# foollh/PicoPose

Hardware: AMD Instinct MI355X
Metric: image-crops/sec (224x224, 162 templates) (higher is better)
Workload: dtype f32 tensors; networks: f32 operands split into 2 f16 terms (22 bits) on f16 MFMA with f32 accumulate; stage-1 contraction: f16 MFMA operands, f32 accumulate, exact f32 re-evaluation of near-ties; PnP f64

## Files before the change

include/picopose_hip.h:

```cpp
#ifndef PICOPOSE_HIP_H
#define PICOPOSE_HIP_H

#include <stddef.h>
#include <stdint.h>

#ifdef __cplusplus
extern "C" {
#endif

#define PP_OK 0
#define PP_EINVAL (-1)
#define PP_EWORKSPACE (-2)
#define PP_ELAUNCH (-3)

#define PP_MATCH_EXACT 0
#define PP_MATCH_FAST 1

const char* pp_strerror(int code);
int pp_version(void);

int pp_prof_enable(int max_records);
int pp_prof_collect(float* out_ms, int max_out, int* count);
int pp_prof_gemm_enable(int max_records);
int pp_prof_gemm_collect(double* ms, double* flops, int* launches);
// ... 97 lines not shown
    const void* B_hl;
    float b_scale;
    const void* A_hl;
    long long a_hl_bytes, b_hl_bytes;
    void* C_hl;
    int ldc_h;
    int c_relu;
    const float* alpha_dev;
    const float* alpha_dev2;
    int ksplit;
    int ks_rows;
    int grp_rows;
    long long grp_b_bytes;
} PpGemmDesc;

int pp_gemm(const PpGemmDesc* desc, void* stream);
int pp_split_f16x3(const float* w, long long n, void* hl, float* scale, void* stream);
int pp_split_weights_ws(const float* w, long long n, int terms, void* out, float* scale2, float* partials, void* stream);
int pp_split_activation(const float* x, long long batch_stride, int B, int P, int row_stride, int C, int relu,
                        void* hl, void* stream);
int pp_split_activation_ld(const float* x, long long batch_stride, int B, int P, int row_stride, int C, int relu,
                           void* hl, int ld_h, void* stream);
int pp_pow2_scale_ws(const float* x, long long n, float* scale2, float* partials, void* stream);
int pp_split_scaled_t(const float* x, long long rows, int ld, int C, const float* scale, void* out, int terms, void* stream);
int pp_split_transpose_t(const float* x, long long rows, int cols, int ld, const float* scale, void* out, int terms, void* stream);
int pp_split_transpose_ld(const float* x, long long rows, int cols, int ld, const float* scale, void* out, long long ld_out, int terms,
                          void* stream);
int pp_im2col_t_operand(const float* x, int B, int H, int W, int C, int ksize, int stride, int pad, void* out, int terms, void* stream);
int pp_sum_slices(const float* part, int S, int M, int N, const float* bias, int act, float* out, void* stream);
int pp_hl_patch_columns(const float* x, int ld_x, int c, long long rows, void* hl, int ld_h, int col0, void* stream);

int pp_split_weights_t(const float* w, long long n, int terms, void* out, float* scale, void* stream);
int pp_split_activation_t(const float* x, long long batch_stride, int B, int P, int row_stride, int C, int relu, void* out,
                          int ld_h, int terms, void* stream);
int pp_hl_patch_columns_t(const float* x, int ld_x, int c, long long rows, void* out, int ld_h, int col0, int terms, void* stream);
int pp_layernorm_t(const float* x, const float* gamma, const float* beta, int rows, int C, float eps, float* y, void* out, int terms,
                   void* stream);
int pp_resize_bilinear_nhwc_t(const float* in, int B, int H, int W, int C, int Ho, int Wo, float mul, void* out, int terms,
                              void* stream);
int pp_resize_bilinear_nhwc_dual(const float* in, int B, int H, int W, int C, int Ho, int Wo, float mul, float* out, void* out_operand,
                                 int terms, void* stream);
int pp_warp_nhwc_t(const float* feat, int feat_batch, const float* flow, int B, int H, int W, int C, int ld_flow, void* out,
                   int ld_h, int terms, void* stream);
int pp_attention_t(const void* qkv_operand, int terms, int B, int T, int heads, int head_dim, float scale, float* out,
                   void* out_operand, void* stream);

int pp_attention(const float* qkv, int B, int T, int heads, int head_dim, float scale, float* out, void* stream);
int pp_attention_split(const float* qkv, int B, int T, int heads, int head_dim, float scale, float* out, void* out_hl,
                       void* stream);
int pp_attention_ex(const float* qkv, int B, int T, int heads, int head_dim, float scale, int prec, float* out, void* out_hl,
                    void* stream);
int pp_attention_hl(const void* qkv_hl, int B, int T, int heads, int head_dim, float scale, float* out, void* out_hl,
                    void* stream);
int pp_attention_train(const float* qkv, int B, int T, int heads, int head_dim, float scale, float* out, float* lse2, void* stream);
int pp_attention_backward(const float* qkv, const float* out, const float* dout, const float* lse2, const float* gpair, int B, int T,
                          int heads, int head_dim, float scale, float* Dws, float* dqkv, void* stream);

int pp_layernorm(const float* x, const float* gamma, const float* beta, int rows, int C, float eps,
                 float* y, void* stream);
int pp_layernorm_split(const float* x, const float* gamma, const float* beta, int rows, int C, float eps, float* y,
                       void* hl, void* stream);
int pp_softmax_rows(float* x, int rows, int n, int ld, void* stream);
int pp_groupnorm_nhwc(const float* x, const float* gamma, const float* beta, int B, int HW, int C,
                      int groups, float eps, int relu, float* y, void* stream);
int pp_transpose_batched(const float* in, long long in_batch_stride, int B, int R, int C, float* out,
                         long long out_batch_stride, int ld_out, int col_off, void* stream);
int pp_assemble_tokens(const float* patches, const float* cls_token, const float* pos, int B, int T, int C,
                       float* tokens, void* stream);
int pp_normalize_rows(const float* x, int rows, int n, float eps, float* y, void* stream);

int pp_resize_bilinear_nhwc(const float* in, int B, int H, int W, int C, int Ho, int Wo, float mul,
                            float* out, void* stream);
int pp_resize_bilinear_nhwc_hl(const float* in, int B, int H, int W, int C, int Ho, int Wo, float mul, void* out_hl,
                               void* stream);
int pp_warp_nhwc(const float* feat, int feat_batch, const float* flow, int B, int H, int W, int C, int ld_flow,
                 float* out, int ld_out, void* stream);
int pp_warp_nhwc_hl(const float* feat, int feat_batch, const float* flow, int B, int H, int W, int C, int ld_flow,
                    void* out_hl, int ld_h, void* stream);
int pp_avgpool2_nhwc(const float* in, int B, int H, int W, int C, float* out, void* stream);
int pp_gather_rows(const float* src, const long long* index, long long n_src_rows, long long row_floats, int n, float* dst,
                   void* stream);
int pp_bank_rows_to_tokens(const float* bank, long long n_bank_rows, int C, int P, const long long* index, int n, float* tokens, int ld,
                           int T, int skip, void* stream);

int pp_crop_resize_normalize(const unsigned char* image, int H, int W, const unsigned char* mask, int y1, int y2, int x1,
                             int x2, int S, int rgb_mask_flag, const double* mean3, const double* std3, float* out_rgb,
                             float* out_mask, void* stream);
int pp_depth_points_nearest(const float* depth_m, int H, int W, int y1, int y2, int x1, int x2, int P, float fx, float fy,
                            float cx, float cy, float* out_pts, void* stream);
int pp_corr_lookup_nhwc(const float* f1, int ld_f1, const float* f2_l0, const float* f2_l1, const float* f2_l2,
                        int f2_batch, const float* flow, int B, int H, int W, int C, int levels, int radius,
                        int ld_flow, float* out, int ld_out, void* stream);
int pp_corr_lookup_nhwc_ex(const float* f1, int ld_f1, const float* f2_l0, const float* f2_l1, const float* f2_l2,
                           int f2_batch, const float* flow, int B, int H, int W, int C, int levels, int radius,
                           int ld_flow, int prec, float* out, int ld_out, void* stream);

int pp_conv_narrow_hl(const void* x_hl, int ld_x, int B, int H, int W, int C, const float* weight, const float* bias, int ksize,
                      int n_out, const float* residual, float* out, void* stream);
int pp_conv_narrow_f32(const float* x, int ld_x, int B, int H, int W, int C, const float* weight, const float* bias, int ksize,
                       int n_out, const float* residual, float* out, void* stream);

int pp_winograd_input_f32(const float* x, int ld_x, long long batch_stride, int B, int H, int W, int C, int relu, float* U, void* stream);
int pp_winograd_weight_f32(const float* w, int Cout, int Cin, int ldw, float* V, void* stream);
int pp_winograd_output_f32(const float* Y, int B, int H, int W, int Cout, const float* bias, int act, const float* residual,
                           const float* residual2, float* out, int ldc, void* stream);

int pp_winograd4_input_hl(const void* x_hl, int ld_x, long long batch_stride, int B, int H, int W, int C, int relu, void* U_hl, long long P_pad,
                          void* stream);
int pp_winograd4_weight_f32(const float* w, int Cout, int Cin, int ldw, float* V, void* stream);
int pp_winograd4_output(const float* Y, int ld_y, int B, int H, int W, int Cout, const float* bias, int act, const float* residual,
                        const float* residual2, float* out, int ldc, void* out_hl, int ld_h, int c_relu, long long P_pad, void* stream);

int pp_winograd4_chain(const float* Y, int ld_y, int B, int H, int W, int C, const float* bias, int act, int c_relu, void* U_hl, long long P_pad,
                       void* stream);

int pp_winograd_chain_f32(const float* Y, int B, int H, int W, int C, const float* bias, int act, int relu_next, float* U, void* stream);

int pp_set_saturation_word(unsigned int* word);

int pp_saturation_take(unsigned int* word, unsigned int* slot, void* stream);


int pp_corr_lookup_nhwc_hl(const void* f1_hl, int ld_f1, const void* f2_hl_l0, const void* f2_hl_l1, const void* f2_hl_l2,
                           int f2_batch, const float* flow, int B, int H, int W, int C, int levels, int radius, int ld_flow,
                           float* out, int ld_out, void* stream);

int pp_pnp_ransac(const float* tar_pts_2d, const float* src_pts_3d, const float* K, const float* tem_pose,
                  const int64_t* tar_pts, const int64_t* src_pts, int P, int H, int W, int N, int iterations,
                  float reproj_threshold, double* rot, double* tvec, double* inlier_ratio, int32_t* success,
                  int32_t* num_points, void* stream);

int pp_pnp_ransac_debug(const float* tar_pts_2d, const float* src_pts_3d, const float* K, const float* tem_pose,
                        const int64_t* tar_pts, const int64_t* src_pts, int P, int H, int W, int N, int iterations,
                        float reproj_threshold, double* rot, double* tvec, double* inlier_ratio, int32_t* success,
                        int32_t* num_points, double* refit_branches, void* stream);

int pp_pnp_ransac_refine(const float* tar_pts_2d, const float* src_pts_3d, const float* K, const float* tem_pose,
                         const int64_t* tar_pts, const int64_t* src_pts, int P, int H, int W, int N, int iterations,
                         float reproj_threshold, int max_iters, double eps, double* rot, double* tvec, double* inlier_ratio,
                         int32_t* success, int32_t* num_points, double* rms_before, double* rms_after, int32_t* lm_iterations,
                         uint8_t* inlier_mask, void* stream);

int pp_pnp_refine_lm(const double* object_points, const double* image_points, const int32_t* count, const double* K,
                     const double* rot_init, const double* tvec_init, int P, int Nmax, int max_iters, double eps, double* rot,
                     double* tvec, double* rms_before, double* rms_after, int32_t* lm_iterations, void* stream);

int pp_rgbd_ransac(const float* tar_pts_2d, const float* src_pts_3d, const float* K, const float* tem_pose,
                   const int64_t* tar_pts, const int64_t* src_pts, int P, int H, int W, int N,
                   const float* depth, int n_images, int dH, int dW, const int32_t* image_index,
                   const float* inlier_dist, int iterations,
                   double* rot, double* tvec, double* inlier_ratio, int32_t* success,
                   int32_t* num_points, int32_t* num_listed, double* rms, uint8_t* inlier_mask, void* stream);

size_t pp_train_keypoints_workspace_bytes(int B);
int pp_train_keypoints(const float* src_mask, const float* tar_mask, int mask_h, int mask_w, const float* src_depth,
                       const float* tar_depth, int depth_h, int depth_w, const float* src_Minv, const float* tar_Minv,
                       const float* src_M, const float* tar_M, const float* src_Kinv, const float* tar_Kinv, const float* src_K,
                       const float* tar_K, const float* T_src2tar, const float* T_tar2src, int B, float* src_pts, float* tar_pts,
                       void* workspace, size_t workspace_bytes, void* stream);
size_t pp_batchnorm_train_workspace_bytes(int rows, int C);
int pp_batchnorm_train(const float* x, const float* gamma, const float* beta, int rows, int C, float eps, float momentum,
                       float* running_mean, float* running_var, int relu, const float* residual, const float* residual2, float* y,
                       void* workspace, size_t workspace_bytes, void* stream);
int pp_gather_normalize_rows(const float* src, long long row_stride, const int64_t* index, int n, int C, float eps, float* out,
                             void* stream);
int pp_xent_diag_rows(const float* logits, int n, int ld, float scale, float* row_loss, void* stream);
// ... 210 lines not shown
```

picopose_amd/_lib.py:

```python
import ctypes
import os
import re

from .build import LIB

_HEADER = os.path.join(os.path.dirname(os.path.abspath(__file__)), "..", "include", "picopose_hip.h")

PP_OK = 0
PP_MATCH_EXACT = 0
PP_MATCH_FAST = 1
PP_BANK_F32 = 0
PP_BANK_F16 = 1

_lib = None


class PpGemmDesc(ctypes.Structure):
    _fields_ = [
        ("A", ctypes.c_void_p), ("B", ctypes.c_void_p), ("C", ctypes.c_void_p), ("bias", ctypes.c_void_p),
        ("gamma", ctypes.c_void_p), ("residual", ctypes.c_void_p), ("residual2", ctypes.c_void_p),
        ("M", ctypes.c_int), ("N", ctypes.c_int), ("K", ctypes.c_int),
        ("lda", ctypes.c_int), ("ldb", ctypes.c_int), ("ldc", ctypes.c_int), ("b_kn", ctypes.c_int),
        ("batch0", ctypes.c_int), ("batch1", ctypes.c_int),
        ("a_bs0", ctypes.c_longlong), ("a_bs1", ctypes.c_longlong), ("b_bs0", ctypes.c_longlong),
# ... 44 lines not shown
            )
        import torch

        L = ctypes.CDLL(LIB)
        c = ctypes
        vp, i32, f32, sz = c.c_void_p, c.c_int, c.c_float, c.c_size_t
        L.pp_strerror.restype = c.c_char_p
        L.pp_strerror.argtypes = [i32]
        L.pp_version.restype = i32
        L.pp_prof_enable.argtypes = [i32]
        L.pp_prof_collect.argtypes = [c.POINTER(f32), i32, c.POINTER(i32)]
        L.pp_prof_gemm_enable.argtypes = [i32]
        L.pp_prof_gemm_collect.argtypes = [c.POINTER(c.c_double), c.POINTER(c.c_double), c.POINTER(i32)]
        L.pp_prof_gemm_records.argtypes = [i32, c.POINTER(i32), c.POINTER(f32), c.POINTER(c.c_double), c.POINTER(i32)]
        L.pp_prof_gemm_records2.argtypes = [i32, c.POINTER(i32), c.POINTER(f32), c.POINTER(c.c_double), c.POINTER(c.c_double), c.POINTER(i32)]
        L.pp_gemm_tune_save.argtypes = [c.c_char_p]
        L.pp_gemm_tune_load.argtypes = [c.c_char_p]
        L.pp_gemm_tune_entries.argtypes = []
        L.pp_gemm_generic_epilogue.argtypes = [i32]
        L.pp_stage1_workspace_bytes.argtypes = [i32, i32, i32, c.POINTER(sz)]
        L.pp_stage1_scores.argtypes = [vp, vp, vp, i32, i32, i32, i32, i32, i32, f32, vp, sz, vp, vp, vp]
        L.pp_stage1_scores_ex.argtypes = [vp, i32, vp, vp, i32, i32, i32, i32, i32, i32, f32, vp, sz, vp, vp, vp]
        L.pp_topk.argtypes = [vp, i32, i32, i32, vp, vp, vp]
        L.pp_stage1_match.argtypes = [vp, vp, vp, i32, i32, i32, i32, i32, i32, i32, f32, vp, sz,
                                      vp, vp, vp, vp, vp]
        L.pp_stage1_match_ex.argtypes = [vp, i32, vp, vp, i32, i32, i32, i32, i32, i32, i32, f32, vp, sz, vp, vp, vp, vp, vp]
        L.pp_stage1_indexed_workspace_bytes.argtypes = [i32, i32, i32, c.POINTER(sz)]
        L.pp_stage1_scores_indexed.argtypes = [vp, i32, vp, i32, vp, vp, i32, i32, i32, i32, i32, i32, f32, vp, sz, vp, vp, vp]
        L.pp_stage1_match_indexed.argtypes = [vp, i32, vp, i32, vp, vp, i32, i32, i32, i32, i32, i32, i32, f32, vp, sz, vp, vp, vp,
                                              vp, vp]
        L.pp_similarity_volume.argtypes = [vp, vp, vp, i32, i32, i32, i32, vp, vp]
        L.pp_calc_pred_Ms.argtypes = [vp, vp, vp, vp, vp, vp, i32, f32, vp, vp]
        L.pp_pose_recovery_2d.argtypes = [vp, vp, vp, vp, vp, vp, i32, vp, vp]
        L.pp_init_correspondences.argtypes = [vp, vp, i32, i32, i32, vp, vp, vp]
        L.pp_stage3_correspondences.argtypes = [vp, vp, i32, i32, i32, f32, vp, vp, vp]
        L.pp_gather_valid.argtypes = [vp, vp, i32, i32, i32, i32, i32, vp, vp, vp]
        L.pp_gemm.argtypes = [c.POINTER(PpGemmDesc), vp]
        L.pp_split_f16x3.argtypes = [vp, c.c_longlong, vp, vp, vp]
        L.pp_split_activation.argtypes = [vp, c.c_longlong, i32, i32, i32, i32, i32, vp, vp]
        L.pp_split_activation_ld.argtypes = [vp, c.c_longlong, i32, i32, i32, i32, i32, vp, i32, vp]
        L.pp_conv_narrow_hl.argtypes = [vp, i32, i32, i32, i32, i32, vp, vp, i32, i32, vp, vp, vp]
        L.pp_conv_narrow_f32.argtypes = [vp, i32, i32, i32, i32, i32, vp, vp, i32, i32, vp, vp, vp]
        L.pp_winograd_input_f32.argtypes = [vp, i32, c.c_longlong, i32, i32, i32, i32, i32, vp, vp]
        L.pp_winograd_weight_f32.argtypes = [vp, i32, i32, i32, vp, vp]
        L.pp_winograd_output_f32.argtypes = [vp, i32, i32, i32, i32, vp, i32, vp, vp, vp, i32, vp]
        L.pp_winograd4_input_hl.argtypes = [vp, i32, c.c_longlong, i32, i32, i32, i32, i32, vp, c.c_longlong, vp]
        L.pp_winograd4_weight_f32.argtypes = [vp, i32, i32, i32, vp, vp]
        L.pp_winograd4_output.argtypes = [vp, i32, i32, i32, i32, i32, vp, i32, vp, vp, vp, i32, vp, i32, i32, c.c_longlong, vp]
        L.pp_winograd4_chain.argtypes = [vp, i32, i32, i32, i32, i32, vp, i32, i32, vp, c.c_longlong, vp]
        L.pp_winograd_chain_f32.argtypes = [vp, i32, i32, i32, i32, vp, i32, i32, vp, vp]
        L.pp_set_saturation_word.argtypes = [vp]
        L.pp_saturation_take.argtypes = [vp, vp, vp]
        L.pp_split_weights_t.argtypes = [vp, c.c_longlong, i32, vp, vp, vp]
        L.pp_split_weights_ws.argtypes = [vp, c.c_longlong, i32, vp, vp, vp, vp]
        L.pp_split_activation_t.argtypes = [vp, c.c_longlong, i32, i32, i32, i32, i32, vp, i32, i32, vp]
        L.pp_hl_patch_columns_t.argtypes = [vp, i32, i32, c.c_longlong, vp, i32, i32, i32, vp]
        L.pp_layernorm_t.argtypes = [vp, vp, vp, i32, i32, f32, vp, vp, i32, vp]
        L.pp_resize_bilinear_nhwc_t.argtypes = [vp, i32, i32, i32, i32, i32, i32, f32, vp, i32, vp]
        L.pp_resize_bilinear_nhwc_dual.argtypes = [vp, i32, i32, i32, i32, i32, i32, f32, vp, vp, i32, vp]
        L.pp_warp_nhwc_t.argtypes = [vp, i32, vp, i32, i32, i32, i32, i32, vp, i32, i32, vp]
        L.pp_attention_t.argtypes = [vp, i32, i32, i32, i32, i32, f32, vp, vp, vp]
        L.pp_sum_slices.argtypes = [vp, i32, i32, i32, vp, i32, vp, vp]
        L.pp_hl_patch_columns.argtypes = [vp, i32, i32, c.c_longlong, vp, i32, i32, vp]
        L.pp_warp_nhwc_hl.argtypes = [vp, i32, vp, i32, i32, i32, i32, i32, vp, i32, vp]
        L.pp_attention.argtypes = [vp, i32, i32, i32, i32, f32, vp, vp]
        L.pp_attention_split.argtypes = [vp, i32, i32, i32, i32, f32, vp, vp, vp]
        L.pp_attention_ex.argtypes = [vp, i32, i32, i32, i32, f32, i32, vp, vp, vp]
        L.pp_attention_hl.argtypes = [vp, i32, i32, i32, i32, f32, vp, vp, vp]
        L.pp_attention_train.argtypes = [vp, i32, i32, i32, i32, f32, vp, vp, vp]
        L.pp_attention_backward.argtypes = [vp, vp, vp, vp, vp, i32, i32, i32, i32, f32, vp, vp, vp]
        L.pp_layernorm.argtypes = [vp, vp, vp, i32, i32, f32, vp, vp]
        L.pp_layernorm_split.argtypes = [vp, vp, vp, i32, i32, f32, vp, vp, vp]
        L.pp_softmax_rows.argtypes = [vp, i32, i32, i32, vp]
        L.pp_groupnorm_nhwc.argtypes = [vp, vp, vp, i32, i32, i32, i32, f32, i32, vp, vp]
        L.pp_transpose_batched.argtypes = [vp, c.c_longlong, i32, i32, i32, vp, c.c_longlong, i32, i32, vp]
        L.pp_assemble_tokens.argtypes = [vp, vp, vp, i32, i32, i32, vp, vp]
        L.pp_normalize_rows.argtypes = [vp, i32, i32, f32, vp, vp]
        L.pp_resize_bilinear_nhwc.argtypes = [vp, i32, i32, i32, i32, i32, i32, f32, vp, vp]
        L.pp_resize_bilinear_nhwc_hl.argtypes = [vp, i32, i32, i32, i32, i32, i32, f32, vp, vp]
        L.pp_warp_nhwc.argtypes = [vp, i32, vp, i32, i32, i32, i32, i32, vp, i32, vp]
        L.pp_avgpool2_nhwc.argtypes = [vp, i32, i32, i32, i32, vp, vp]
        L.pp_gather_rows.argtypes = [vp, vp, c.c_longlong, c.c_longlong, i32, vp, vp]
        L.pp_bank_rows_to_tokens.argtypes = [vp, c.c_longlong, i32, i32, vp, i32, vp, i32, i32, i32, vp]
        L.pp_depth_points_nearest.argtypes = [vp, i32, i32, i32, i32, i32, i32, i32, f32, f32, f32, f32, vp, vp]
        L.pp_crop_resize_normalize.argtypes = [vp, i32, i32, vp, i32, i32, i32, i32, i32, i32, c.POINTER(c.c_double),
                                               c.POINTER(c.c_double), vp, vp, vp]
        L.pp_corr_lookup_nhwc.argtypes = [vp, i32, vp, vp, vp, i32, vp, i32, i32, i32, i32, i32, i32, i32, vp, i32, vp]
        L.pp_corr_lookup_nhwc_ex.argtypes = [vp, i32, vp, vp, vp, i32, vp, i32, i32, i32, i32, i32, i32, i32, i32, vp, i32, vp]
        L.pp_corr_lookup_nhwc_hl.argtypes = [vp, i32, vp, vp, vp, i32, vp, i32, i32, i32, i32, i32, i32, i32, vp, i32, vp]
        L.pp_pnp_ransac.argtypes = [vp, vp, vp, vp, vp, vp, i32, i32, i32, i32, i32, f32, vp, vp, vp, vp, vp, vp]
        L.pp_pnp_ransac_debug.argtypes = [vp, vp, vp, vp, vp, vp, i32, i32, i32, i32, i32, f32, vp, vp, vp, vp, vp, vp, vp]
        L.pp_pnp_ransac_refine.argtypes = [vp, vp, vp, vp, vp, vp, i32, i32, i32, i32, i32, f32, i32, c.c_double] + [vp] * 10
        L.pp_pnp_refine_lm.argtypes = [vp] * 6 + [i32, i32, i32, c.c_double] + [vp] * 6
        L.pp_rgbd_ransac.argtypes = [vp] * 6 + [i32] * 4 + [vp, i32, i32, i32, vp, vp, i32] + [vp] * 9
        L.pp_train_keypoints_workspace_bytes.restype = sz
        L.pp_train_keypoints_workspace_bytes.argtypes = [i32]
        L.pp_train_keypoints.argtypes = [vp, vp, i32, i32, vp, vp, i32, i32] + [vp] * 10 + [i32, vp, vp, vp, sz, vp]
        L.pp_batchnorm_train_workspace_bytes.restype = sz
        L.pp_batchnorm_train_workspace_bytes.argtypes = [i32, i32]
        L.pp_batchnorm_train.argtypes = [vp, vp, vp, i32, i32, f32, f32, vp, vp, i32, vp, vp, vp, vp, sz, vp]
        L.pp_gather_normalize_rows.argtypes = [vp, c.c_longlong, vp, i32, i32, f32, vp, vp]
        L.pp_xent_diag_rows.argtypes = [vp, i32, i32, f32, vp, vp]
        L.pp_flow_loss_blocks.argtypes = []
        L.pp_flow_loss_sums.argtypes = [vp, vp, vp, i32, i32, i32, f32, vp, vp]
        ll = c.c_longlong
        L.pp_colsum_workspace_bytes.restype = sz
        L.pp_colsum_workspace_bytes.argtypes = [ll, i32]
        L.pp_colsum.argtypes = [vp, ll, i32, i32, vp, vp, sz, vp]
        L.pp_act_forward.argtypes = [vp, ll, i32, vp, vp]
        L.pp_act_backward.argtypes = [vp, vp, ll, i32, vp, vp]
        L.pp_elementwise.argtypes = [i32, vp, vp, ll, i32, vp, vp]
        L.pp_layernorm_backward.argtypes = [vp, vp, vp, i32, i32, f32, vp, vp, vp]
        L.pp_groupnorm_backward_nhwc.argtypes = [vp, vp, vp, vp, i32, i32, i32, i32, f32, i32, vp, vp, vp, vp]
        L.pp_softmax_backward_rows.argtypes = [vp, vp, ll, i32, vp, vp]
        L.pp_xent_diag_backward.argtypes = [vp, i32, i32, f32, vp, vp, vp]
        L.pp_normalize_rows_backward.argtypes = [vp, ll, vp, vp, i32, i32, f32, vp, vp]
        L.pp_scatter_add_rows.argtypes = [vp, vp, i32, i32, vp, vp]
        L.pp_im2col_nhwc.argtypes = [vp, i32, i32, i32, i32, i32, i32, i32, vp, vp]
        L.pp_col2im_nhwc.argtypes = [vp, i32, i32, i32, i32, i32, i32, i32, vp, vp]
        L.pp_simvol_backward.argtypes = [vp, vp, vp, i32, i32, i32, vp, vp]
        L.pp_im2col_t_nhwc.argtypes = [vp, i32, i32, i32, i32, i32, i32, i32, vp, vp]
        L.pp_pow2_scale.argtypes = [vp, ll, vp, vp]
        L.pp_pow2_scale_ws.argtypes = [vp, ll, vp, vp, vp]
        L.pp_split_scaled_t.argtypes = [vp, ll, i32, i32, vp, vp, i32, vp]
        L.pp_split_transpose_t.argtypes = [vp, ll, i32, i32, vp, vp, i32, vp]
        L.pp_split_transpose_ld.argtypes = [vp, ll, i32, i32, vp, vp, ll, i32, vp]
        L.pp_im2col_t_operand.argtypes = [vp, i32, i32, i32, i32, i32, i32, i32, vp, i32, vp]
        L.pp_split_with_scale_t.argtypes = [vp, ll, i32, vp, vp, vp]
        L.pp_batchnorm_train_backward_workspace_bytes.restype = sz
        L.pp_batchnorm_train_backward_workspace_bytes.argtypes = [ll, i32]
        L.pp_batchnorm_train_backward.argtypes = [vp, vp, vp, vp, ll, i32, f32, i32, vp, vp, vp, vp, sz, vp]
        L.pp_resize_bilinear_backward_nhwc.argtypes = [vp, i32, i32, i32, i32, i32, i32, f32, vp, vp]
        L.pp_avgpool2_backward_nhwc.argtypes = [vp, i32, i32, i32, i32, i32, vp, vp]
        L.pp_warp_backward_nhwc.argtypes = [vp, vp, vp, i32, i32, i32, i32, i32, vp, vp, vp]
        L.pp_corr_lookup_backward_nhwc.argtypes = [vp, vp, vp, vp, i32, i32, i32, i32, i32, i32, i32, i32, vp, vp, vp, vp]
        L.pp_warp_backward_nhwc_fixed.argtypes = [vp, vp, vp, i32, i32, i32, i32, i32, vp, vp, vp]
        L.pp_corr_lookup_backward_nhwc_fixed.argtypes = [vp, vp, vp, vp, i32, i32, i32, i32, i32, i32, i32, i32, vp, vp, vp, vp]
        L.pp_fixed_to_float.argtypes = [vp, ll, vp, vp]
        L.pp_flow_loss_backward.argtypes = [vp, vp, vp, i32, i32, i32, f32, vp, vp, vp, vp, vp]
        L.pp_adam_workspace_bytes.argtypes = [c.POINTER(PpAdamTensor), i32, c.POINTER(sz)]
        L.pp_adam_multi_tensor.argtypes = [c.POINTER(PpAdamTensor), i32, vp, i32, i32, vp, sz, vp]
        L.pp_augment_execute.argtypes = [vp, vp, ll, vp, ll, vp, i32, vp, i32, vp, c.POINTER(i32), i32, vp, vp, ll, vp, vp]
        L.pp_augment_resize.argtypes = [vp, vp, ll, vp, i32, i32, i32, c.POINTER(c.c_double), c.POINTER(c.c_double), vp, vp, vp]
        L.pp_depth_u16_scaled.argtypes = [vp, ll, i32, vp, vp, vp]
        L.pp_depth_u16_template.argtypes = [vp, ll, vp, vp]
        L.pp_detections_crop.argtypes = [vp, i32, i32, vp, i32, vp, vp, c.POINTER(i32), c.POINTER(i32), i32, i32, i32,
                                         c.POINTER(c.c_double), c.POINTER(c.c_double), vp, vp, vp]
        L.pp_render_workspace_bytes.argtypes = [i32, i32, i32, i32, c.POINTER(sz)]
        L.pp_render_views.argtypes = [vp, i32, vp, vp, i32, vp, vp, i32, f32, f32, f32, f32, i32, i32, f32, vp, sz, vp, vp, vp, vp, vp, vp]
        L.pp_texture_mips_bytes.argtypes = [i32, i32, c.POINTER(sz), c.POINTER(i32)]
        L.pp_texture_build_mips.argtypes = [vp, i32, i32, vp, sz, vp]
        L.pp_render_views_textured.argtypes = [vp, i32, vp, vp, i32, vp, vp, i32, i32, vp, i32, f32, f32, f32, f32, i32, i32, f32, vp, sz,
                                               vp, vp, vp, vp, vp, vp]
        L.pp_vertex_normals.argtypes = [vp, i32, vp, i32, vp, vp, vp, vp]
        L.pp_render_views_lit.argtypes = [vp, i32, vp, vp, i32, vp, vp, vp, i32, i32, vp, i32, f32, f32, f32, f32, i32, i32, f32, vp, sz,
                                          vp, vp, vp, vp, vp, vp, i32, f32, i32, vp, vp, vp, i32, vp]
        L.pp_template_extents.argtypes = [vp, i32, i32, i32, vp, vp, vp]
        L.pp_templates_crop.argtypes = [vp, vp, i32, i32, i32, i32, vp, vp, f32, f32, f32, f32, i32, i32, i32,
                                        c.POINTER(c.c_double), c.POINTER(c.c_double), vp, vp, vp, vp]
        L.pp_pose_errors_workspace_bytes.argtypes = [i32, i32, i32, i32, c.POINTER(sz)]
        L.pp_pose_errors.argtypes = [vp] * 10 + [i32] + [vp] * 7 + [i32, i32, vp, sz] + [vp] * 7
        L.pp_vsd_workspace_bytes.argtypes = [ll, ll, c.POINTER(sz)]
        scene = c.POINTER(PpScene)
        L.pp_vsd_errors.argtypes = [scene, vp, vp, vp, vp, i32, vp, f32, vp, i32, vp, sz, vp, vp, vp, vp, vp]
        L.pp_depth_refine_workspace_bytes.argtypes = [ll, ll, ll, c.POINTER(sz)]
        L.pp_depth_refine.argtypes = [scene, vp, vp, vp, vp, vp, i32, f32, i32, f32, f32, f32, f32, f32, vp, sz,
# ... 37 lines not shown
```

picopose_amd/csrc/pp_gemm.hip:

```cpp

#include <hip/hip_runtime.h>
#include <stdint.h>
#include <stdio.h>
#include <stdlib.h>
#include <atomic>
#include <mutex>
#include <string>
#include <unordered_map>
#include "../../include/picopose_hip.h"
#include "pp_common.h"
#include "pp_gemm_dev.h"
#include "pp_gemm_u.h"

static std::mutex g_tune_mu;
static std::unordered_map<std::string, int> g_tune_best;
static int g_tune_loaded = 0;

static int tune_load_locked(const char* path) {
    FILE* f = fopen(path, "r");
    if (!f) return -1;
    char key[192];
    int cfg, n = 0;
    while (fscanf(f, "%191s %d", key, &cfg) == 2) {
        g_tune_best[key] = cfg;
// ... 1068 lines not shown
        PpGemmDesc g = d;
        g.grp_rows = d.M;
        g.grp_b_bytes = d.b_bs0 * 4;
        g.M = d.M * d.batch0;
        g.batch0 = 1;
        if (pp_gemm_f_ok(g)) d = g;
    }
    if (d.A_hl && d.B_hl && d.batch0 > 1 && d.batch1 == 1 && d.conv_kh == 0 && !d.b_kn && d.shuffle_r == 0 && !d.residual && !d.residual2 &&
        d.ksplit <= 1 && !d.C_hl && d.M % 256 == 0 && d.a_bs0 == (long long)d.M * d.lda && d.c_bs0 == (long long)d.M * d.ldc &&
        (long long)d.M * d.batch0 < (1LL << 31) && d.b_bs0 >= 0 && d.b_bs0 % 8 == 0) {
        d.grp_rows = d.M;
        d.grp_b_bytes = d.b_bs0 * (d.prec == PP_PREC_F16 ? 2 : 4);
        d.M *= d.batch0;
        d.batch0 = 1;
    }
    const long long z = v.z = (long long)d.batch0 * d.batch1;
    const bool f16 = d.prec == PP_PREC_F16;
    const int terms = v.terms = f16 ? 1 : 2;
    const bool split = v.split = d.prec == PP_PREC_F16X3 && vec;
    const bool asplit = v.asplit = d.A_hl != nullptr;
    if (f16 && !asplit) return PP_EINVAL;
    if (asplit) {
        const bool ok = d.B_hl && (d.prec == PP_PREC_F16X3 || f16) && z == 1 && !d.b_kn && !d.relu_in &&
                        d.K % 8 == 0 && d.lda % 8 == 0 && d.ldb % 8 == 0 && d.b_scale > 0.f &&
                        (d.conv_kh == 0 || (d.conv_cin % 8 == 0 && d.conv_bstride % 8 == 0)) &&
                        ((uintptr_t)d.A_hl % 16 == 0) && ((uintptr_t)d.B_hl % 16 == 0);
        if (!ok) return PP_EINVAL;
        pp_gemm_extents(d, 2 * terms, d.a_hl_bytes, d.b_hl_bytes);
        if (d.a_hl_bytes >= 0xFFFFFF00LL || d.b_hl_bytes >= 0xFFFFFF00LL) return PP_EINVAL;
    }
    d.ks_rows = 0;
    if (d.ksplit > 1) {
        if (!asplit || d.conv_kh != 0 || d.M % 256 != 0 || d.K % (64 * d.ksplit) != 0 || d.bias || d.gamma || d.residual || d.residual2 ||
            d.act != 0 || d.C_hl || d.shuffle_r != 0 || !d.C || (long long)d.M * d.ksplit >= (1LL << 31))
            return PP_EINVAL;
        d.ks_rows = d.M;
        d.M *= d.ksplit;
        d.K /= d.ksplit;
    }
    if (d.B_hl && (d.b_kn || d.ldb % 8 != 0 || d.K % 8 != 0 || z != 1 || !(d.b_scale > 0.f))) return PP_EINVAL;
    if (d.B_hl && !split && !f16) {
        if (d.alpha_dev || d.alpha_dev2) return PP_EINVAL;
        d.B_hl = nullptr;
    }
    v.fvec = f_engine_on && !asplit && !split && vec && z == 1 && pp_gemm_f_ok(d);
    if (v.fvec) pp_gemm_extents(d, 4, d.a_hl_bytes, d.b_hl_bytes);
    v.u_vec = asplit && pp_gemm_u_vec_ok(d);
    v.h_shape = v.u_vec && pp_gemm_uh_shape_ok(d, terms);
    return PP_OK;
}

static int tail_rows(const GemmView& v, int big_bn, int cus) {
    const PpGemmDesc& d = v.d;
    if (!((v.asplit || v.fvec) && d.conv_kh == 0 && d.shuffle_r == 0 && d.ks_rows == 0 && d.grp_rows == 0 && v.z == 1)) return 0;
    const long long gx = (d.N + big_bn - 1) / big_bn, gy = (d.M + 255) / 256, tiles = gx * gy, full = tiles / cus;
    if (full < 1 || tiles % cus == 0) return 0;
    const long long r = full * cus / gx * 256;
    return (r > 0 && r < d.M && d.M - r >= 128) ? (int)r : 0;
}

enum { GE_U, GE_UH, GE_F, GE_FLY, GE_R1 };
struct GemmPlan {
    int engine;
    int cfg;
    int tile;
    int amode;
    bool vec;
    int tail_rows;
};

static GemmPlan gemm_plan(const GemmView& v, int cfg, int cus) {
    const PpGemmDesc& d = v.d;
    GemmPlan p{};
    if (cfg == 9 || cfg == 10) {
        p.tail_rows = cfg == 10 || d.N > 128 ? tail_rows(v, cfg == 9 ? 256 : 128, cus) : 0;
        cfg = cfg == 9 ? 5 : 4;
    }
    if (v.asplit) {
        cfg = cfg == 3 ? 4 : (cfg == 1 || cfg == 7 || cfg == 8) ? 0 : cfg;
        if (cfg == 6 && !(v.h_shape && d.N > 128)) cfg = 5;
        if (cfg == 5 && d.N <= 128) cfg = 4;
        if (!v.u_vec && cfg != 2) cfg = 0;
        p.engine = cfg == 6 ? GE_UH : GE_U;
        p.tile = cfg == 5 ? PP_U_256x256 : cfg == 4 ? PP_U_256x128 : cfg == 2 ? PP_U_128x64 : PP_U_128x128;
        p.amode = cfg == 6 ? 1 : pp_gemm_u_mode(d, v.terms);
        p.vec = v.u_vec;
    } else if (v.fvec && (cfg >= 3 || d.grp_rows != 0)) {
        if (cfg < 3) cfg = 3;
        const int mode = pp_gemm_f_mode(d);
        if (mode == 2 && (cfg == 5 || cfg == 7)) cfg = 4;
        p.engine = GE_F;
        p.tile = cfg == 7 ? PP_F_256x192 : cfg == 5 ? PP_U_256x256 : cfg == 4 ? PP_U_256x128 : cfg == 3 ? PP_U_128x128 : PP_U_128x64;
        p.amode = 16 + mode;
    } else {
        p.engine = v.split ? GE_FLY : GE_R1;
        p.amode = 8 + (v.vec ? 1 : 0) + (v.split ? 2 : 0);
        p.vec = v.vec;
    }
    p.cfg = cfg;
    return p;
}

static int gemm_r1_launch(const GemmPlan& p, const PpGemmDesc& d, long long z, hipStream_t st) {
    const bool narrow = p.cfg == 2, occ2 = p.cfg == 0;
    void (*k)(PpGemmDesc);
    if (p.engine == GE_FLY && d.B_hl) k = narrow ? gemm_f16x3_kernel<1, 4, true> : occ2 ? gemm_f16x3_kernel<2, 2, true> : gemm_f16x3_kernel<2, 3, true>;
    else if (p.engine == GE_FLY) k = narrow ? gemm_f16x3_kernel<1, 4, false> : occ2 ? gemm_f16x3_kernel<2, 2, false> : gemm_f16x3_kernel<2, 3, false>;
    else if (!p.vec) k = narrow ? gemm_kernel<false, 1, 2> : gemm_kernel<false, 2, 2>;
    else k = narrow ? gemm_kernel<true, 1, 4> : occ2 ? gemm_kernel<true, 2, 2> : gemm_kernel<true, 2, 3>;
    const dim3 grid((d.N + (narrow ? 63 : 127)) / (narrow ? 64 : 128), (unsigned)((d.M + BM - 1) / BM), (unsigned)z);
    void* args[] = {(void*)&d};
    (void)hipLaunchKernel((const void*)k, grid, dim3(256), args, 0, st);
    return PP_OK;
}

static int gemm_launch(const GemmPlan& p, const GemmView& v, int cus, hipStream_t st) {
    auto one = [&](const PpGemmDesc& d, int tile) {
        switch (p.engine) {
            case GE_U: return (v.terms == 2 ? pp_gemm_u_launch_t2 : pp_gemm_u_launch_t1)(d, tile, p.amode, p.vec, cus, st);
            case GE_UH: return pp_gemm_uh_launch(d, v.terms, cus, st);
            case GE_F: return pp_gemm_f_launch(d, tile, p.amode - 16, cus, st);
            default: return gemm_r1_launch(p, d, v.z, st);
        }
    };
    if (p.tail_rows == 0) return one(v.d, p.tile);
    auto rows = [&](int r0, int m) {
        PpGemmDesc t = v.d;
        t.M = m;
        const size_t eb = v.terms == 1 ? 2 : 4;
        if (t.A_hl) t.A_hl = (const char*)t.A_hl + (size_t)r0 * t.lda * eb;
        if (t.A) t.A += (size_t)r0 * t.lda;
        if (t.C) t.C += (size_t)r0 * t.ldc;
        if (t.C_hl) t.C_hl = (char*)t.C_hl + (size_t)r0 * t.ldc_h * eb;
        if (t.residual) t.residual += (size_t)r0 * t.ldc;
        if (t.residual2) t.residual2 += (size_t)r0 * t.ldc;
        pp_gemm_extents(t, (int)eb, t.a_hl_bytes, t.b_hl_bytes);
        return t;
    };
    const int rc = one(rows(0, p.tail_rows), p.tile);
    return rc != PP_OK ? rc : one(rows(p.tail_rows, v.d.M - p.tail_rows), PP_U_128x128);
}

static int tune_candidates(const GemmView& v, int cus, int* c) {
    static const int tail_env = [] { const char* e = getenv("PP_GEMM_TAIL_SPLIT"); return e ? (e[0] == '1' ? 1 : 0) : -1; }();
    const PpGemmDesc& d = v.d;
    const bool tail_on = tail_env == 1, tail_on_f = tail_env != 0;
    const long long t4 = (long long)((d.M + 255) / 256) * ((d.N + 127) / 128), t5 = (long long)((d.M + 255) / 256) * ((d.N + 255) / 256);
    int n = 0;
    if (v.asplit) {
        c[n++] = 0;
        c[n++] = 2;
        if (t4 >= cus / 2) c[n++] = 4;
        if (t5 >= cus / 2 && d.N > 128) c[n++] = 5;
        if (t5 >= cus / 2 && d.N > 128 && v.h_shape) c[n++] = 6;
        if (tail_on && d.N > 128 && tail_rows(v, 256, cus)) c[n++] = 9;
        if (tail_on && tail_rows(v, 128, cus)) c[n++] = 10;
    } else if (v.fvec) {
        c[n++] = 6;
        if (d.N > 64) c[n++] = 3;
        if (t4 >= cus / 2 && d.N > 64) c[n++] = 4;
        if (t5 >= cus / 2 && d.N > 128) c[n++] = 5;
        if ((d.N + 191) / 192 * 192 - d.N < (d.N + 127) / 128 * 128 - d.N && (long long)((d.M + 255) / 256) * ((d.N + 191) / 192) >= cus / 2) c[n++] = 7;
        if (tail_on_f && d.N > 128 && tail_rows(v, 256, cus)) c[n++] = 9;
        if (tail_on_f && d.N > 64 && tail_rows(v, 128, cus)) c[n++] = 10;
    } else {
        for (int i = 0; i < (v.vec ? 3 : 2); ++i) c[n++] = v.vec ? i : (i == 0 ? 0 : 2);
    }
    return n;
}

static int gemm_tune(const GemmView& v, const char* key, int cus, hipStream_t st) {
    static const bool dbg = getenv("PP_GEMM_DEBUG") != nullptr;
    hipEvent_t e0, e1;
    PP_CHECK_HIP(hipEventCreate(&e0));
    PP_CHECK_HIP(hipEventCreate(&e1));
    int cands[12];
    const int nc = tune_candidates(v, cus, cands);
    GemmPlan plans[12];
    float ms[12];
    for (int i = 0; i < nc; ++i) {
        plans[i] = gemm_plan(v, cands[i], cus);
        ms[i] = 1e30f;
        (void)gemm_launch(plans[i], v, cus, st);
    }
    for (int rep = 0; rep < 4; ++rep)
        for (int i = 0; i < nc; ++i) {
            (void)hipEventRecord(e0, st);
            for (int k = 0; k < 4; ++k) (void)gemm_launch(plans[i], v, cus, st);
            (void)hipEventRecord(e1, st);
            (void)hipEventSynchronize(e1);
            float t = 0.f;
            (void)hipEventElapsedTime(&t, e0, e1);
            ms[i] = t < ms[i] ? t : ms[i];
        }
    (void)hipEventDestroy(e0);
    (void)hipEventDestroy(e1);
    int best = 0;
    for (int i = 0; i < nc; ++i) {
        if (dbg) fprintf(stderr, "[pp_gemm] autotune %s cfg %d: %.4f ms\n", key, cands[i], ms[i]);
        if (ms[i] < ms[best]) best = i;
    }
    g_tune_best[key] = cands[best];
    const int rc = gemm_launch(plans[best], v, cus, st);
    return rc != PP_OK ? rc : pp_last_launch();
}

extern "C" {

int pp_gemm_generic_epilogue(int on) {
    if (on != 0 && on != 1) return PP_EINVAL;
    return g_epi_generic.exchange(on);
}

int pp_gemm(const PpGemmDesc* desc, void* stream) {
    GemmView v;
    if (const int rc = gemm_normalise(desc, v); rc != PP_OK) return rc;
    const PpGemmDesc& d = v.d;
    hipStream_t st = (hipStream_t)stream;
    const int cus = pp_cu_count();
    int cfg = v.fvec ? (d.N <= 64 ? 6 : 3) : (d.N <= 64 ? 2 : 0);
    bool pinned = false;
    if (const char* f = getenv("PP_GEMM_FORCE_CFG")) {
        const int fc = atoi(f);
        if (((fc == 9 || fc == 10) && (v.asplit || v.fvec)) || (fc >= 0 && fc <= 8 && (v.asplit || fc <= 2 || (v.fvec && fc <= 7)))) {
            cfg = fc;
            pinned = true;
        }
    }
    const bool alias = d.C != nullptr && (d.residual == d.C || d.residual2 == d.C);
    static const bool tune = [] { const char* e = getenv("PP_GEMM_AUTOTUNE"); return !(e && e[0] == '0'); }();
    if (!pinned && tune && !alias && (d.N > 64 || v.fvec)) {
        [[maybe_unused]] static const bool env_loaded = [] {
            if (const char* p = getenv("PP_GEMM_TUNE_FILE")) {
                std::lock_guard<std::mutex> lock(g_tune_mu);
                (void)tune_load_locked(p);
            }
            return true;
        }();
        char key[160];
        snprintf(key, sizeof key, "%d.%d.%d.%d.%d.%lld.%d.%d.%d.%d.%d.%d", d.M, d.N, d.K, (int)v.vec, d.b_kn, v.z, d.conv_kh,
                 d.conv_cin, d.conv_stride, d.conv_h, d.shuffle_r,
                 (int)v.split + 2 * (d.B_hl != nullptr) + 4 * (int)v.asplit + 8 * (int)(v.terms == 1) + 16 * (int)v.fvec);
        std::lock_guard<std::mutex> lock(g_tune_mu);
        auto it = g_tune_best.find(key);
        if (it == g_tune_best.end()) return gemm_tune(v, key, cus, st);
        cfg = it->second;
    }
    const GemmPlan p = gemm_plan(v, cfg, cus);
    PpGemmProf* gp = pp_gemm_prof_state();
    const bool rec = gp->capacity > 0 && gp->count < gp->capacity;
    if (rec) (void)hipEventRecord(gp->ev[2 * gp->count], st);
    const int rc = gemm_launch(p, v, cus, st);
    if (rec) {
        (void)hipEventRecord(gp->ev[2 * gp->count + 1], st);
        gp->flops[gp->count] = 2.0 * d.M * d.N * d.K * (double)v.z;
        const double eb = 2.0 * v.terms, ea = v.asplit ? eb : 4.0, ew = (v.asplit || d.B_hl) ? eb : 4.0;
        const long long per = (long long)d.conv_ho * d.conv_wo;
        const double a_el = d.conv_kh != 0 ? (double)((d.M + per - 1) / per) * d.conv_h * d.conv_w * d.conv_cin
                                           : (double)d.M * d.K;
        const double mn = (double)d.M * d.N;
        gp->bytes[gp->count] = (double)v.z * (a_el * ea + (double)d.N * d.K * ew * (d.grp_rows ? d.M / d.grp_rows : 1) + (d.C ? mn * 4.0 : 0.0) +
                                              (d.C_hl ? mn * eb : 0.0) + (d.residual ? mn * 4.0 : 0.0) + (d.residual2 ? mn * 4.0 : 0.0));
        gp->kind[gp->count] = p.engine == GE_U || p.engine == GE_UH ? 0 : 1;
        int* sh = gp->shape[gp->count];
        sh[0] = d.M, sh[1] = d.N, sh[2] = d.K, sh[3] = d.conv_kh, sh[4] = p.cfg, sh[5] = p.amode;
        gp->count++;
    }
    return rc != PP_OK ? rc : pp_last_launch();
}

int pp_gemm_tune_save(const char* path) {
    if (!path) return PP_EINVAL;
    std::lock_guard<std::mutex> lock(g_tune_mu);
    FILE* f = fopen(path, "w");
    if (!f) return PP_EINVAL;
    for (const auto& kv : g_tune_best) fprintf(f, "%s %d\n", kv.first.c_str(), kv.second);
    fclose(f);
    return (int)g_tune_best.size();
}

int pp_gemm_tune_load(const char* path) {
    if (!path) return PP_EINVAL;
    std::lock_guard<std::mutex> lock(g_tune_mu);
    const int n = tune_load_locked(path);
    return n < 0 ? PP_EINVAL : n;
}

int pp_gemm_tune_entries(void) {
    std::lock_guard<std::mutex> lock(g_tune_mu);
    return (int)g_tune_best.size();
}

int pp_layernorm(const float* x, const float* gamma, const float* beta, int rows, int C, float eps, float* y,
                 void* stream) {
    if (!x || !gamma || !beta || !y || rows <= 0 || C <= 0) return PP_EINVAL;
    launch_layernorm(x, gamma, beta, rows, C, eps, y, nullptr, (hipStream_t)stream);
    return pp_last_launch();
}

int pp_layernorm_t(const float* x, const float* gamma, const float* beta, int rows, int C, float eps, float* y,
                   void* hl, int terms, void* stream) {
    if (!x || !gamma || !beta || !hl || rows <= 0 || C <= 0 || C % 8 != 0 || (terms != 1 && terms != 2)) return PP_EINVAL;
    launch_layernorm(x, gamma, beta, rows, C, eps, y, (_Float16*)hl, (hipStream_t)stream, terms);
    return pp_last_launch();
}

int pp_layernorm_split(const float* x, const float* gamma, const float* beta, int rows, int C, float eps, float* y,
// ... 46 lines not shown
```

picopose_amd/csrc/pp_gemm_u.h:

```cpp
#ifndef PP_GEMM_U_H
#define PP_GEMM_U_H
#include <hip/hip_runtime.h>
#include "../../include/picopose_hip.h"

enum { PP_U_128x64 = 0, PP_U_128x128 = 1, PP_U_256x128 = 2, PP_U_256x256 = 3, PP_F_256x192 = 4  };

int pp_gemm_u_mode(const PpGemmDesc& d, int terms);
int pp_gemm_u_launch_t1(const PpGemmDesc& d, int tile, int mode, bool vec, int cus, hipStream_t st);
int pp_gemm_u_launch_t2(const PpGemmDesc& d, int tile, int mode, bool vec, int cus, hipStream_t st);
bool pp_gemm_uh_shape_ok(const PpGemmDesc& d, int terms);
bool pp_gemm_u_vec_ok(const PpGemmDesc& d);
int pp_gemm_epi_kind(const PpGemmDesc& d);
int pp_gemm_uh_launch(const PpGemmDesc& d, int terms, int cus, hipStream_t st);
bool pp_gemm_f_ok(const PpGemmDesc& d);
int pp_gemm_f_mode(const PpGemmDesc& d);
int pp_gemm_f_launch(const PpGemmDesc& d, int tile, int mode, int cus, hipStream_t st);

static inline void pp_gemm_extents(const PpGemmDesc& d, int eb, long long& a, long long& b) {
    const long long per = (long long)d.conv_ho * d.conv_wo;
    a = eb * (d.conv_kh != 0 ? ((d.M + per - 1) / per - 1) * d.conv_bstride + (long long)d.conv_h * d.conv_w * d.lda : (long long)(d.M - 1) * d.lda + d.K);
    b = eb * ((long long)(d.N - 1) * d.ldb + d.K + (d.grp_rows != 0 ? (long long)(d.M / d.grp_rows - 1) * d.b_bs0 : 0));
}
#endif
```

picopose_amd/csrc/pp_gemm_u_kernel.h:

```cpp
#ifndef PP_GEMM_U_KERNEL_H
#define PP_GEMM_U_KERNEL_H
#include <hip/hip_runtime.h>
#include <stdint.h>
#include <type_traits>
#include "pp_gemm_dev.h"
#include "pp_gemm_u.h"

typedef __attribute__((address_space(3))) void* lds_ptr_t;
#ifdef PP_STUDY_OFFMASK
#define PP_STUDY_OFF(x) ((x) & (unsigned)(PP_STUDY_OFFMASK))
#else
#define PP_STUDY_OFF(x) (x)
#endif

#ifndef PP_U1_BAND_ROWS
#define PP_U1_BAND_ROWS 4
#endif

template <int BM_, int BN_, int WM_, int WN_, int S_, int OCC_, int PREF_ = 0, int B3_ = 0>
struct TileCfg {
    static constexpr int BM = BM_, BN = BN_, WM = WM_, WN = WN_, S = S_, OCC = OCC_;
    static constexpr bool PREF = PREF_ != 0;
    static constexpr bool B3 = B3_ != 0;
    static constexpr int NW = WM_ * WN_;
// ... 758 lines not shown
    int cab = 0;
    load_a(fa0, 0, -1, 0);
    load_b(fb0, 0, 0);
    int cur = 0;
    const float descale = pp_alpha(d) / (PP_A_SCALE * d.b_scale);
    for (int tile = first; tile < chunk1; tile += nxw) {
#pragma unroll
        for (int i = 0; i < MI; ++i)
#pragma unroll
            for (int j = 0; j < NJ; ++j) acc[i][j] = f32x4{0.f, 0.f, 0.f, 0.f};
#define PP_H_STEP(DX, NDX, NAB)                                                                                       \
        {                                                                                                             \
            load_b(fb1, cur, 1);                                                                                      \
            load_a(fa1, cab, DX, 1);                                                                                  \
            mma_unit(fa0, fb0, 0, 0);                                                                                 \
            __builtin_amdgcn_sched_barrier(0);                                                                        \
            mma_unit(fa0, fb1, 0, 1);                                                                                 \
            __builtin_amdgcn_sched_barrier(0);                                                                        \
            load_a(fa0, cab, DX, 2);                                                                                  \
            mma_unit(fa1, fb0, 1, 0);                                                                                 \
            __builtin_amdgcn_sched_barrier(0);                                                                        \
            mma_unit(fa1, fb1, 1, 1);                                                                                 \
            __builtin_amdgcn_sched_barrier(0);                                                                        \
            load_a(fa1, cab, DX, 3);                                                                                  \
            mma_unit(fa0, fb0, 2, 0);                                                                                 \
            __builtin_amdgcn_sched_barrier(0);                                                                        \
            mma_unit(fa0, fb1, 2, 1);                                                                                 \
            __builtin_amdgcn_sched_barrier(0);                                                                        \
            mma_unit(fa1, fb0, 3, 0);                                                                                 \
            __builtin_amdgcn_sched_barrier(0);                                                                        \
                                            \
            asm volatile("s_waitcnt vmcnt(0) lgkmcnt(0)" ::: "memory");                                               \
            __builtin_amdgcn_s_barrier();                                                                             \
                                                                                                            \
            PP_H_NEXT_TILE_IF_DONE()                                                                                  \
            const int nst = cur ^ 1;                                                                                  \
            if (DX == 0) dma_a(0);                                                                                    \
            load_a(fa0, NAB, NDX, 0);                                                                                 \
            mma1(fa1, fb1, 3, 1, 0, 0);                                                                               \
            __builtin_amdgcn_sched_barrier(0);                                                                        \
            if (DX == 0) { dma_a(1); dma_a(2); }                                                                      \
            load_b(fb0, nst, 0);                                                                                      \
            mma1(fa1, fb1, 3, 1, 0, 1);                                                                               \
            __builtin_amdgcn_sched_barrier(0);                                                                        \
            if (DX == 0) { dma_a(3); if (five) dma_a(4); }                                                            \
            dma_b(cur, 0);                                                                                            \
            mma1(fa1, fb1, 3, 1, 1, 0);                                                                               \
            __builtin_amdgcn_sched_barrier(0);                                                                        \
            dma_b(cur, 1);                                                                                            \
            dma_b(cur, 2);                                                                                            \
            __builtin_amdgcn_sched_barrier(0);                                                                        \
            dma_b(cur, 3);                                                                                            \
            PP_H_ADVANCE()                                                                                            \
            mma1(fa1, fb1, 3, 1, 1, 1);                                                                               \
            cur = nst;                                                                                                \
        }
        for (int kt = 0; kt < nk; kt += 3) {
            PP_H_STEP(-1, 0, cab)
            PP_H_STEP(0, 1, cab)
            PP_H_STEP(1, -1, cab ^ 1)
            cab ^= 1;
        }
#undef PP_H_STEP
        {
            int tr, tc;
            pp_tile_rc_g(tile, gx, gy, 8, TERMS == 1 ? PP_U1_BAND_ROWS : 4, tr, tc);
            const int mw = tr * H_BM + wr * 128, nw = tc * H_BN + wc * 64;
            if (VEC) epilogue_wave16<MI, NJ, TERMS>(d, descale, acc, mw, nw, lane);
            else epilogue_scalar16<MI, NJ, TERMS>(d, descale, acc, mw, nw, lane);
        }
        __builtin_amdgcn_s_waitcnt(0x0F70);
    }
    asm volatile("s_waitcnt vmcnt(0)" ::: "memory");
#undef PP_H_SETUP
#undef PP_H_NEXT_TILE_IF_DONE
#undef PP_H_ADVANCE
#endif
}

typedef TileCfg<256, 256, 2, 4, 2, 1, 0, 1> T256x256;
typedef TileCfg<256, 128, 4, 2, 3, 1, 1> T256x128;
typedef TileCfg<128, 128, 2, 2, 2, 2> T128x128;
typedef TileCfg<128, 64, 2, 2, 3, 2> T128x64;

template <class T, int MODE, int TERMS, bool VEC, int EPI = PP_EPI_GENERIC>
static int pp_u_launch_one(const PpGemmDesc& d, int persistent_slots, hipStream_t st) {
    static signed char attr_state[PP_MAX_DEVICES];
    signed char& ok = attr_state[pp_cur_device()];
    if (ok == 0)
        ok = hipFuncSetAttribute((const void*)pp_gemm_u_kernel<T, MODE, TERMS, VEC, EPI>, hipFuncAttributeMaxDynamicSharedMemorySize, T::LDS_BYTES) == hipSuccess ? 1 : -1;
    if (ok < 0) return PP_ELAUNCH;
    const int gx = (d.N + T::BN - 1) / T::BN, gy = (d.M + T::BM - 1) / T::BM;
    const int nt = gx * gy;
    const int g = nt < persistent_slots ? (nt + 7) / 8 * 8 : persistent_slots / 8 * 8;
    hipLaunchKernelGGL((pp_gemm_u_kernel<T, MODE, TERMS, VEC, EPI>), dim3(g), dim3(T::NW * 64), T::LDS_BYTES, st, d, gx, gy);
    return PP_OK;
}

template <class T, int TERMS, bool VEC>
static int pp_u_launch_tile(const PpGemmDesc& d, int mode, int slots, hipStream_t st) {
    if constexpr (VEC && TERMS == 2 && (std::is_same<T, T256x256>::value || std::is_same<T, T256x128>::value)) {
        if (mode == 0) {
            switch (pp_gemm_epi_kind(d)) {
                case PP_EPI_HL_LIN: return pp_u_launch_one<T, 0, TERMS, VEC, PP_EPI_HL_LIN>(d, slots, st);
                case PP_EPI_HL_GELU: return pp_u_launch_one<T, 0, TERMS, VEC, PP_EPI_HL_GELU>(d, slots, st);
                case PP_EPI_C_BGR: return pp_u_launch_one<T, 0, TERMS, VEC, PP_EPI_C_BGR>(d, slots, st);
                case PP_EPI_C_PLAIN: return pp_u_launch_one<T, 0, TERMS, VEC, PP_EPI_C_PLAIN>(d, slots, st);
                default: break;
            }
        }
    }
    if (mode == 0) return pp_u_launch_one<T, 0, TERMS, VEC>(d, slots, st);
    if (mode == 1) return pp_u_launch_one<T, 1, TERMS, VEC>(d, slots, st);
    if (mode == 3) {
        if constexpr (TERMS == 2 && VEC) return pp_u_launch_one<T, 3, TERMS, VEC>(d, slots, st);
        else return PP_EINVAL;
    }
    return pp_u_launch_one<T, 2, TERMS, VEC>(d, slots, st);
}

template <int TERMS>
static int pp_u_launch_terms(const PpGemmDesc& d, int tile, int mode, bool vec, int cus, hipStream_t st) {
    if (!vec) {
        if (tile == PP_U_128x64) return pp_u_launch_tile<T128x64, TERMS, false>(d, mode, 2 * cus, st);
        if (tile == PP_U_128x128) return pp_u_launch_tile<T128x128, TERMS, false>(d, mode, 2 * cus, st);
        return PP_EINVAL;
    }
    switch (tile) {
        case PP_U_256x256: return pp_u_launch_tile<T256x256, TERMS, true>(d, mode, cus, st);
        case PP_U_256x128: return pp_u_launch_tile<T256x128, TERMS, true>(d, mode, cus, st);
        case PP_U_128x128: return pp_u_launch_tile<T128x128, TERMS, true>(d, mode, 2 * cus, st);
        case PP_U_128x64: return pp_u_launch_tile<T128x64, TERMS, true>(d, mode, 2 * cus, st);
        default: return PP_EINVAL;
    }
}
#endif
```

picopose_amd/csrc/pp_sample.hip:

```cpp

#include <hip/hip_runtime.h>
#include <stdlib.h>
#include <stdint.h>
#include "../../include/picopose_hip.h"
#include "pp_common.h"
#include "pp_crop_dev.h"

namespace {

typedef float f4 __attribute__((ext_vector_type(4)));

__device__ __forceinline__ float resize_blend(float a, float b, float c, float d, float hx, float lx, float hy, float ly, float mul) {
#pragma clang fp contract(off)
    const float top = fmaf(hx, a, lx * b), bot = fmaf(hx, c, lx * d);
    return (hy * top + ly * bot) * mul;
}

__global__ __launch_bounds__(256) void resize_kernel(const float* __restrict__ in, int H, int W, int C,
                                                     int Ho, int Wo, float mul, float* __restrict__ out,
                                                     _Float16* __restrict__ out_hl, int terms) {
    const int b = blockIdx.z, oy = blockIdx.y, tid = threadIdx.x;
    const float sy = Ho > 1 ? (float)(H - 1) / (float)(Ho - 1) : 0.f;
    const float sx = Wo > 1 ? (float)(W - 1) / (float)(Wo - 1) : 0.f;
    const float fy = sy * (float)oy;
// ... 121 lines not shown
                                                       float* __restrict__ out) {
    const int Ho = H / 2, Wo = W / 2, b = blockIdx.y;
    const size_t n = (size_t)Ho * Wo * C;
    const float* ib = in + (size_t)b * H * W * C;
    float* ob = out + (size_t)b * n;
    for (size_t i = (size_t)blockIdx.x * 256 + threadIdx.x; i < n; i += (size_t)gridDim.x * 256) {
        const int c = (int)(i % C);
        const size_t q = i / C;
        const int ox = (int)(q % Wo), oy = (int)(q / Wo);
        const float* p = ib + ((size_t)(2 * oy) * W + 2 * ox) * C + c;
        ob[i] = ((p[0] + p[C]) + (p[(size_t)W * C] + p[(size_t)W * C + C])) * 0.25f;
    }
}

constexpr int MAXR = 2, TW = 2 * MAXR + 2, MAXL = 3;
__global__ __launch_bounds__(256) void corr_lookup_kernel(const float* __restrict__ f1, int ld_f1,
                                                          int f2_batch, const float* __restrict__ f2l0,
                                                          const float* __restrict__ f2l1,
                                                          const float* __restrict__ f2l2,
                                                          const float* __restrict__ flow, int H, int W, int C,
                                                          int L, int r, int ld_flow, float inv_sqrt_c,
                                                          float* __restrict__ out, int ld_out) {
    extern __shared__ __attribute__((aligned(16))) float sm[];
    const int wv = threadIdx.x >> 6, lane = threadIdx.x & 63;
    float* a = sm + (size_t)wv * (C + MAXL * TW * TW);
    float* tab = a + C;
    const int b = blockIdx.y, p = blockIdx.x * 4 + wv;
    const bool live = p < H * W;
    const int y = live ? p / W : 0, x = live ? p - y * W : 0;
    const int tw = 2 * r + 2, win = 2 * r + 1;
    if (live) {
        const float* src = f1 + ((size_t)b * H * W + p) * ld_f1;
        for (int c = lane * 4; c < C; c += 256) *(f4*)(a + c) = *(const f4*)(src + c);
    }
    __builtin_amdgcn_fence(__ATOMIC_RELEASE, "wavefront");
    __builtin_amdgcn_s_waitcnt(0xC07F);
    __builtin_amdgcn_wave_barrier();
    float cx[MAXL], cy[MAXL];
    int bx[MAXL], by[MAXL];
    if (live) {
        const float* fl = flow + ((size_t)b * H * W + p) * ld_flow;
        const float gx = (float)x + fl[0], gy = (float)y + fl[1];
        for (int l = 0; l < L; ++l) {
            const int Hl = H >> l, Wl = W >> l;
            const float sc = (float)(1 << l);
            cx[l] = fminf(fmaxf(roundtrip(gx / sc, Wl), -(float)(r + 2)), (float)(Wl + r + 1));
            cy[l] = fminf(fmaxf(roundtrip(gy / sc, Hl), -(float)(r + 2)), (float)(Hl + r + 1));
            bx[l] = (int)floorf(cx[l]) - r;
            by[l] = (int)floorf(cy[l]) - r;
        }
        const int npos = L * tw * tw;
        for (int i = lane; i < npos; i += 64) {
            const int l = i / (tw * tw), rem = i - l * tw * tw, dy = rem / tw, dx = rem - dy * tw;
            const int Hl = H >> l, Wl = W >> l;
            const int qx = bx[l] + dx, qy = by[l] + dy;
            float dot = 0.f;
            const bool inside = qx >= 0 && qx < Wl && qy >= 0 && qy < Hl;
            const int qxc = min(max(qx, 0), Wl - 1), qyc = min(max(qy, 0), Hl - 1);
            const float* f2 = l == 0 ? f2l0 : (l == 1 ? f2l1 : f2l2);
            const float* q = f2 + (((size_t)(b % f2_batch) * Hl + qyc) * Wl + qxc) * C;
            for (int c = 0; c < C; c += 4) {
                const f4 u = *(const f4*)(a + c), v = *(const f4*)(q + c);
                dot = fmaf(u.x, v.x, dot);
                dot = fmaf(u.y, v.y, dot);
                dot = fmaf(u.z, v.z, dot);
                dot = fmaf(u.w, v.w, dot);
            }
            tab[i] = inside ? dot * inv_sqrt_c : 0.f;
        }
    }
    __builtin_amdgcn_fence(__ATOMIC_RELEASE, "wavefront");
    __builtin_amdgcn_s_waitcnt(0xC07F);
    __builtin_amdgcn_wave_barrier();
    if (live) {
        float* o = out + ((size_t)b * H * W + p) * ld_out;
        const int nout = L * win * win;
        for (int i = lane; i < nout; i += 64) {
            const int l = i / (win * win), rem = i - l * win * win, ai = rem / win, bi = rem - ai * win;
            const float wx1 = cx[l] - floorf(cx[l]), wy1 = cy[l] - floorf(cy[l]);
            const float wx0 = 1.f - wx1, wy0 = 1.f - wy1;
            const float* t = tab + l * tw * tw + bi * tw + ai;
            o[i] = t[0] * (wx0 * wy0) + t[1] * (wx1 * wy0) + t[tw] * (wx0 * wy1) + t[tw + 1] * (wx1 * wy1);
        }
    }
}

constexpr int CT = 8, CM = CT * CT;
constexpr int CRW = 16, CN = CRW * CRW;
constexpr int CK = 32, CKP = CK + 4;
typedef _Float16 h8_t __attribute__((ext_vector_type(8)));
typedef _Float16 h4_t __attribute__((ext_vector_type(4)));
constexpr int CSP = CN + 4;
typedef float f32x16_t __attribute__((ext_vector_type(16)));

template <bool HLIN, bool EXACT = false, bool ONE = false>
__global__ __launch_bounds__(256, 2) void corr_lookup_mfma_kernel(const void* __restrict__ f1v, int ld_f1, int f2_batch,
                                                                  const void* __restrict__ f2l0, const void* __restrict__ f2l1,
                                                                  const void* __restrict__ f2l2, const float* __restrict__ flow,
                                                                  int B, int H, int W, int C, int L, int r, int ld_flow,
                                                                  float inv_sqrt_c, float* __restrict__ out, int ld_out) {
    extern __shared__ __attribute__((aligned(16))) float sm[];
    float* As = sm;
    float* Bs = sm + CM * CKP;
    float* S = sm;
    __shared__ float s_cx[CM], s_cy[CM];
    __shared__ int s_bx[CM], s_by[CM], s_state[CM], s_ox, s_oy, s_todo;
    const int tid = threadIdx.x, lane = tid & 63, wv = tid >> 6, l31 = lane & 31, lh = lane >> 5;
    const int tiles_x = W / CT, tiles = tiles_x * (H / CT), total = tiles * B;
    int g = blockIdx.x;
    if (total % 8 == 0) g = (g % 8) * (total / 8) + g / 8;
    const int b = g / tiles, tile = g - b * tiles;
    const int y0 = (tile / tiles_x) * CT, x0 = (tile % tiles_x) * CT;
    const int tw = 2 * r + 2, win = 2 * r + 1, fit = CRW - tw;
    const int my = tid >> 3, mx = tid & 7;
    float gx = 0.f, gy = 0.f;
    if (tid < CM) {
        const float* fl = flow + ((size_t)b * H * W + (size_t)(y0 + my) * W + x0 + mx) * ld_flow;
        gx = (float)(x0 + mx) + fl[0];
        gy = (float)(y0 + my) + fl[1];
    }
    for (int l = 0; l < L; ++l) {
        const int Hl = H >> l, Wl = W >> l;
        const void* f2v = l == 0 ? f2l0 : (l == 1 ? f2l1 : f2l2);
        const float* f2 = (const float*)f2v + (size_t)(b % f2_batch) * Hl * Wl * C;
        const _Float16* f2h = (const _Float16*)f2v + (size_t)(b % f2_batch) * Hl * Wl * C * 2;
        const float* f1 = (const float*)f1v;
        const _Float16* f1h = (const _Float16*)f1v;
        if (tid == 0) s_todo = 0;
        __syncthreads();
        if (tid < CM) {
            const float sc = (float)(1 << l);
            const float cx = fminf(fmaxf(roundtrip(gx / sc, Wl), -1.0e6f), 1.0e6f);
            const float cy = fminf(fmaxf(roundtrip(gy / sc, Hl), -1.0e6f), 1.0e6f);
            const int bx = (int)floorf(cx) - r, by = (int)floorf(cy) - r;
            s_cx[tid] = cx; s_cy[tid] = cy; s_bx[tid] = bx; s_by[tid] = by;
            const bool outside = bx >= Wl || by >= Hl || bx + tw <= 0 || by + tw <= 0;
            s_state[tid] = outside ? 2 : 0;
            if (!outside) atomicAdd(&s_todo, 1);
        }
        __syncthreads();
        for (int idx = tid; idx < CM * win * win; idx += 256) {
            const int m = idx / (win * win), o = idx - m * (win * win);
            if (s_state[m] == 2)
                out[((size_t)b * H * W + (size_t)(y0 + (m >> 3)) * W + x0 + (m & 7)) * ld_out + l * win * win + o] = 0.f;
        }
        while (s_todo > 0) {
            if (tid == 0) { s_ox = 0x7fffffff; s_oy = 0x7fffffff; }
            __syncthreads();
            if (tid < CM && s_state[tid] == 0) atomicMin(&s_ox, s_bx[tid]);
            __syncthreads();
            if (tid < CM && s_state[tid] == 0 && s_bx[tid] - s_ox <= fit) atomicMin(&s_oy, s_by[tid]);
            __syncthreads();
            const int ox = s_ox, oy = s_oy;
            f32x16_t acc[2][2];
#pragma unroll
            for (int i = 0; i < 2; ++i)
#pragma unroll
                for (int j = 0; j < 2; ++j)
#pragma unroll
                    for (int e = 0; e < 16; ++e) acc[i][j][e] = 0.f;
            f4 ra0[2], rb0[8], ra1[2], rb1[8];
            const int part = tid & 7, row0 = tid >> 3;
            auto load_chunk = [&](int kc, f4 (&ra)[2], f4 (&rb)[8]) __attribute__((always_inline)) {
#pragma unroll
                for (int i = 0; i < 2; ++i) {
                    const int m = row0 + 32 * i;
                    const size_t px = (size_t)b * H * W + (size_t)(y0 + (m >> 3)) * W + x0 + (m & 7);
                    ra[i] = HLIN ? *(const f4*)(f1h + (px * ld_f1 + kc * CK) * 2 + 8 * part) : *(const f4*)(f1 + px * ld_f1 + kc * CK + 4 * part);
                }
#pragma unroll
                for (int i = 0; i < 8; ++i) {
                    const int n = row0 + 32 * i, qy = oy + (n >> 4), qx = ox + (n & 15);
                    const bool in = qx >= 0 && qx < Wl && qy >= 0 && qy < Hl;
                    const size_t px = (size_t)qy * Wl + qx;
                    rb[i] = !in ? f4{0.f, 0.f, 0.f, 0.f}
                                : (HLIN ? *(const f4*)(f2h + (px * C + kc * CK) * 2 + 8 * part) : *(const f4*)(f2 + px * C + kc * CK + 4 * part));
                }
            };
            auto put = [&](float* rowp, f4 v) __attribute__((always_inline)) {
                if (EXACT) {
                    *(f4*)(rowp + 4 * part) = v;
                    return;
                }
                if (HLIN) {
                    *(f4*)((_Float16*)rowp + 8 * part) = v;
                    return;
                }
                _Float16* g8 = (_Float16*)rowp + 16 * (part >> 1) + 4 * (part & 1);
                if (ONE) {
                    const h4_t hi = {pp_to_f16(v.x), pp_to_f16(v.y), pp_to_f16(v.z), pp_to_f16(v.w)};
                    *(h4_t*)g8 = hi;
                    return;
                }
                _Float16 h0, h1, h2, h3, l0, l1, l2, l3;
                pp_split_f16(v.x, h0, l0);
                pp_split_f16(v.y, h1, l1);
                pp_split_f16(v.z, h2, l2);
                pp_split_f16(v.w, h3, l3);
                const h4_t hi = {h0, h1, h2, h3}, lo = {l0, l1, l2, l3};
                *(h4_t*)g8 = hi;
                *(h4_t*)(g8 + 8) = lo;
            };
#ifdef PP_STUDY_CORR_NK1
// ... 174 lines not shown

constexpr int NRW_PITCH = 144;

template <int KS, int NOUT, bool F32IN = false>
__global__ __launch_bounds__(256) void conv_narrow_kernel(const _Float16* __restrict__ x, int ldx, int H, int W, int C,
                                                          const float* __restrict__ w, const float* __restrict__ bias,
                                                          const float* __restrict__ residual, float* __restrict__ out) {
    constexpr int R = KS / 2;
    extern __shared__ __attribute__((aligned(16))) unsigned char nsm[];
    const int TH = 256 / W, bands = H / TH;
    const int b = blockIdx.x / bands, y0 = (blockIdx.x % bands) * TH;
    const int tid = threadIdx.x, ty = tid / W, tx = tid % W;
    const int PW = W + 2 * R, PH = TH + 2 * R;
    float acc[NOUT];
#pragma unroll
    for (int n = 0; n < NOUT; ++n) acc[n] = 0.f;
    const int K = KS * KS * C;
    constexpr int MAXP = F32IN ? 13 : 7, PPX = F32IN ? 8 : 4;
    const int npiece = PH * PW * PPX;
    float4 pre[F32IN ? MAXP : 2 * MAXP];
    auto fetch = [&](int c0) __attribute__((always_inline)) {
#pragma unroll
        for (int j = 0; j < MAXP; ++j) {
            const int i = min(tid + 256 * j, npiece - 1);
            const int piece = i % PPX, px = i / PPX, sy = px / PW, sx = px - sy * PW;
            const int iy = y0 + sy - R, ix = sx - R;
            const unsigned m = 0u - (unsigned)((tid + 256 * j < npiece) & (iy >= 0) & (iy < H) & (ix >= 0) & (ix < W));
            const int iyc = min(max(iy, 0), H - 1), ixc = min(max(ix, 0), W - 1);
            typedef unsigned u4n __attribute__((ext_vector_type(4)));
            if constexpr (F32IN) {
                const u4n raw = *(const u4n*)((const float*)x + (((size_t)b * H + iyc) * W + ixc) * (size_t)ldx + c0 + 4 * piece) & m;
                pre[j] = __builtin_bit_cast(float4, raw);
            } else {
                const u4n* src = (const u4n*)(x + (((size_t)b * H + iyc) * W + ixc) * (size_t)(2 * ldx) + 2 * c0 + 16 * piece);
                pre[2 * j] = __builtin_bit_cast(float4, src[0] & m);
                pre[2 * j + 1] = __builtin_bit_cast(float4, src[1] & m);
            }
        }
    };
    fetch(0);
    for (int c0 = 0; c0 < C; c0 += 32) {
        __syncthreads();
#pragma unroll
        for (int j = 0; j < MAXP; ++j) {
            const int i = tid + 256 * j;
            if (i >= npiece) continue;
            if constexpr (F32IN) {
                *(float4*)(nsm + (size_t)(i >> 3) * NRW_PITCH + 16 * (i & 7)) = pre[j];
            } else {
                typedef _Float16 h8v __attribute__((ext_vector_type(8)));
                const h8v hi = __builtin_bit_cast(h8v, pre[2 * j]), lo = __builtin_bit_cast(h8v, pre[2 * j + 1]);
                float4 a, c;
                a.x = (float)hi[0] + (float)lo[0]; a.y = (float)hi[1] + (float)lo[1]; a.z = (float)hi[2] + (float)lo[2]; a.w = (float)hi[3] + (float)lo[3];
                c.x = (float)hi[4] + (float)lo[4]; c.y = (float)hi[5] + (float)lo[5]; c.z = (float)hi[6] + (float)lo[6]; c.w = (float)hi[7] + (float)lo[7];
                unsigned char* d = nsm + (size_t)(i >> 2) * NRW_PITCH + 32 * (i & 3);
                *(float4*)d = a;
                *(float4*)(d + 16) = c;
            }
        }
        __syncthreads();
        if (c0 + 32 < C) fetch(c0 + 32);
#pragma unroll
        for (int dy = 0; dy < KS; ++dy)
#pragma unroll
            for (int dx = 0; dx < KS; ++dx) {
                const unsigned char* p = nsm + (size_t)((ty + dy) * PW + tx + dx) * NRW_PITCH;
                const float* wt = w + (dy * KS + dx) * C + c0;
#pragma unroll
                for (int g = 0; g < 8; ++g) {
                    const f4 xv = *(const f4*)(p + 16 * g);
#pragma unroll
                    for (int e = 0; e < 4; ++e)
#pragma unroll
                        for (int n = 0; n < NOUT; ++n) acc[n] = fmaf(xv[e], wt[n * K + 4 * g + e], acc[n]);
                }
            }
    }
    const size_t o = (((size_t)b * H + y0 + ty) * W + tx) * NOUT;
#pragma unroll
    for (int n = 0; n < NOUT; ++n) {
        float v = (F32IN ? acc[n] : acc[n] * (1.0f / PP_A_SCALE)) + (bias ? bias[n] : 0.f);
        if (residual) v += residual[o + n];
        out[o + n] = v;
    }
}

}

PP_SAT_SETTER(pp_sat_set_sample)

extern "C" {

int pp_resize_bilinear_nhwc(const float* in, int B, int H, int W, int C, int Ho, int Wo, float mul, float* out,
                            void* stream) {
    if (!in || !out || B <= 0 || H <= 0 || W <= 0 || C <= 0 || Ho <= 0 || Wo <= 0) return PP_EINVAL;
    const bool vec = (C & 3) == 0 && (((uintptr_t)in | (uintptr_t)out) & 15) == 0;
    const int work = vec ? Wo * (C / 4) : Wo * C;
    const int gx = (work + 1023) / 1024;
    hipLaunchKernelGGL(resize_kernel, dim3(gx < 64 ? gx : 64, Ho, B), dim3(256), 0, (hipStream_t)stream, in, H, W,
                       C, Ho, Wo, mul, out, (_Float16*)nullptr, 2);
    return pp_last_launch();
}

int pp_resize_bilinear_nhwc_t(const float* in, int B, int H, int W, int C, int Ho, int Wo, float mul, void* out_hl,
                              int terms, void* stream) {
    if (!in || !out_hl || B <= 0 || H <= 0 || W <= 0 || C <= 0 || C % 8 != 0 || Ho <= 0 || Wo <= 0 ||
        (((uintptr_t)in | (uintptr_t)out_hl) & 15) != 0 || (terms != 1 && terms != 2))
        return PP_EINVAL;
    const int gx = (Wo * (C / 8) + 1023) / 1024;
    hipLaunchKernelGGL(resize_kernel, dim3(gx < 64 ? gx : 64, Ho, B), dim3(256), 0, (hipStream_t)stream, in, H, W,
                       C, Ho, Wo, mul, (float*)nullptr, (_Float16*)out_hl, terms);
    return pp_last_launch();
}

int pp_resize_bilinear_nhwc_dual(const float* in, int B, int H, int W, int C, int Ho, int Wo, float mul, float* out, void* out_hl,
                                 int terms, void* stream) {
    if (!in || !out || !out_hl || B <= 0 || H <= 0 || W <= 0 || C <= 0 || C % 8 != 0 || Ho <= 0 || Wo <= 0 ||
        (((uintptr_t)in | (uintptr_t)out | (uintptr_t)out_hl) & 15) != 0 || (terms != 1 && terms != 2))
        return PP_EINVAL;
    const int gx = (Wo * (C / 8) + 1023) / 1024;
    hipLaunchKernelGGL(resize_kernel, dim3(gx < 64 ? gx : 64, Ho, B), dim3(256), 0, (hipStream_t)stream, in, H, W,
                       C, Ho, Wo, mul, out, (_Float16*)out_hl, terms);
    return pp_last_launch();
}

int pp_resize_bilinear_nhwc_hl(const float* in, int B, int H, int W, int C, int Ho, int Wo, float mul, void* out_hl,
                               void* stream) {
    return pp_resize_bilinear_nhwc_t(in, B, H, W, C, Ho, Wo, mul, out_hl, 2, stream);
}

int pp_warp_nhwc(const float* feat, int feat_batch, const float* flow, int B, int H, int W, int C, int ld_flow,
                 float* out, int ld_out, void* stream) {
    if (!feat || !flow || !out || B <= 0 || H <= 0 || W <= 0 || C <= 0 || C % 4 != 0 || ld_flow < 2 || feat_batch <= 0 ||
        ld_out < C || ld_out % 4 != 0 || ((uintptr_t)out % 16) != 0)
        return PP_EINVAL;
    hipLaunchKernelGGL(warp_kernel<false>, dim3((H * W + 3) / 4, B), dim3(256), 0, (hipStream_t)stream, feat, feat_batch, flow,
                       H, W, C, ld_flow, out, ld_out, 2);
    return pp_last_launch();
}

int pp_warp_nhwc_t(const float* feat, int feat_batch, const float* flow, int B, int H, int W, int C, int ld_flow,
                   void* out_hl, int ld_h, int terms, void* stream) {
    if (!feat || !flow || !out_hl || B <= 0 || H <= 0 || W <= 0 || C <= 0 || C % 8 != 0 || ld_flow < 2 || feat_batch <= 0 ||
        ld_h < C || ld_h % 8 != 0 || ((uintptr_t)out_hl % 16) != 0 || (terms != 1 && terms != 2))
        return PP_EINVAL;
    hipLaunchKernelGGL(warp_kernel<true>, dim3((H * W + 3) / 4, B), dim3(256), 0, (hipStream_t)stream, feat, feat_batch, flow,
                       H, W, C, ld_flow, (float*)out_hl, ld_h, terms);
    return pp_last_launch();
}

int pp_warp_nhwc_hl(const float* feat, int feat_batch, const float* flow, int B, int H, int W, int C, int ld_flow,
                    void* out_hl, int ld_h, void* stream) {
    return pp_warp_nhwc_t(feat, feat_batch, flow, B, H, W, C, ld_flow, out_hl, ld_h, 2, stream);
}

int pp_avgpool2_nhwc(const float* in, int B, int H, int W, int C, float* out, void* stream) {
    if (!in || !out || B <= 0 || H < 2 || W < 2 || C <= 0 || H % 2 != 0 || W % 2 != 0) return PP_EINVAL;
    const size_t n = (size_t)(H / 2) * (W / 2) * C;
    const int gx = (int)((n + 255) / 256 < 1024 ? (n + 255) / 256 : 1024);
    hipLaunchKernelGGL(avgpool2_kernel, dim3(gx, B), dim3(256), 0, (hipStream_t)stream, in, H, W, C, out);
    return pp_last_launch();
}

static int corr_tiled_launch(bool hl, const void* f1, int ld_f1, const void* f2_l0, const void* f2_l1, const void* f2_l2, int f2_batch,
                             const float* flow, int B, int H, int W, int C, int levels, int radius, int ld_flow, float* out, int ld_out,
                             void* stream, bool exact = false, bool one = false) {
// ... 31 lines not shown
    const int TH = 256 / W, R = ksize / 2;
    const size_t lds = (size_t)(TH + 2 * R) * (W + 2 * R) * NRW_PITCH;
    const dim3 grid((unsigned)(B * (H / TH)));
    hipStream_t st = (hipStream_t)stream;
#define NRW_LAUNCH(KS_, N_)                                                                                                                  \
    hipLaunchKernelGGL((conv_narrow_kernel<KS_, N_, true>), grid, dim3(256), lds, st, (const _Float16*)x, ld_x, H, W, C, weight, bias, residual, out)
    if (ksize == 3 && n_out == 2) NRW_LAUNCH(3, 2);
    else if (ksize == 3) NRW_LAUNCH(3, 1);
    else if (n_out == 2) NRW_LAUNCH(1, 2);
    else NRW_LAUNCH(1, 1);
#undef NRW_LAUNCH
    return pp_last_launch();
}

int pp_corr_lookup_nhwc_ex(const float* f1, int ld_f1, const float* f2_l0, const float* f2_l1, const float* f2_l2,
                           int f2_batch, const float* flow, int B, int H, int W, int C, int levels, int radius,
                           int ld_flow, int prec, float* out, int ld_out, void* stream) {
    if (prec != PP_PREC_F32 && prec != PP_PREC_F16X3 && prec != PP_PREC_F16) return PP_EINVAL;
    if (!f1 || !f2_l0 || !flow || !out || B <= 0 || H <= 0 || W <= 0 || C <= 0 || C % 4 != 0) return PP_EINVAL;
    if (ld_f1 < C || ld_f1 % 4 != 0 || ((uintptr_t)f1 % 16) != 0 || f2_batch <= 0) return PP_EINVAL;
    if (levels < 1 || levels > MAXL || radius < 1 || radius > MAXR) return PP_EINVAL;
    if ((levels > 1 && !f2_l1) || (levels > 2 && !f2_l2)) return PP_EINVAL;
    if ((H >> (levels - 1)) < 1 || (W >> (levels - 1)) < 1 || ld_flow < 2) return PP_EINVAL;
    const int win = 2 * radius + 1;
    if (ld_out < levels * win * win) return PP_EINVAL;
    const char* te = getenv("PP_CORR_TILED");
    const bool tiled = !(te && te[0] == '0');
    const bool aligned = (((uintptr_t)f2_l0 | (levels > 1 ? (uintptr_t)f2_l1 : 0) | (levels > 2 ? (uintptr_t)f2_l2 : 0)) % 16) == 0;
    if (tiled && H % CT == 0 && W % CT == 0 && C % CK == 0 && aligned)
        return corr_tiled_launch(false, f1, ld_f1, f2_l0, f2_l1, f2_l2, f2_batch, flow, B, H, W, C, levels, radius, ld_flow, out, ld_out, stream,
                                 prec == PP_PREC_F32, prec == PP_PREC_F16);
    const size_t smem = (size_t)4 * (C + MAXL * TW * TW) * sizeof(float);
    hipLaunchKernelGGL(corr_lookup_kernel, dim3((H * W + 3) / 4, B), dim3(256), smem, (hipStream_t)stream, f1, ld_f1,
                       f2_batch, f2_l0, f2_l1, f2_l2, flow, H, W, C, levels, radius, ld_flow, 1.0f / sqrtf((float)C), out,
                       ld_out);
    return pp_last_launch();
}

int pp_corr_lookup_nhwc_hl(const void* f1_hl, int ld_f1, const void* f2_hl_l0, const void* f2_hl_l1, const void* f2_hl_l2,
                           int f2_batch, const float* flow, int B, int H, int W, int C, int levels, int radius, int ld_flow,
                           float* out, int ld_out, void* stream) {
    if (!f1_hl || !f2_hl_l0 || !flow || !out || B <= 0 || H <= 0 || W <= 0 || C <= 0 || f2_batch <= 0) return PP_EINVAL;
    if (H % CT != 0 || W % CT != 0 || C % CK != 0 || ld_f1 < C || ld_f1 % 8 != 0) return PP_EINVAL;
    if (((uintptr_t)f1_hl | (uintptr_t)f2_hl_l0 | (uintptr_t)f2_hl_l1 | (uintptr_t)f2_hl_l2) % 16 != 0) return PP_EINVAL;
    if (levels < 1 || levels > MAXL || radius < 1 || radius > MAXR) return PP_EINVAL;
    if ((levels > 1 && !f2_hl_l1) || (levels > 2 && !f2_hl_l2)) return PP_EINVAL;
    if ((H >> (levels - 1)) < 1 || (W >> (levels - 1)) < 1 || ld_flow < 2) return PP_EINVAL;
    const int win = 2 * radius + 1;
    if (ld_out < levels * win * win) return PP_EINVAL;
    return corr_tiled_launch(true, f1_hl, ld_f1, f2_hl_l0, f2_hl_l1, f2_hl_l2, f2_batch, flow, B, H, W, C, levels, radius, ld_flow, out, ld_out,
                             stream);
}

int pp_corr_lookup_nhwc(const float* f1, int ld_f1, const float* f2_l0, const float* f2_l1, const float* f2_l2,
                        int f2_batch, const float* flow, int B, int H, int W, int C, int levels, int radius,
                        int ld_flow, float* out, int ld_out, void* stream) {
    return pp_corr_lookup_nhwc_ex(f1, ld_f1, f2_l0, f2_l1, f2_l2, f2_batch, flow, B, H, W, C, levels, radius, ld_flow,
                                  PP_PREC_F16X3, out, ld_out, stream);
}

int pp_gather_rows(const float* src, const long long* index, long long n_src_rows, long long row_floats, int n, float* dst,
                   void* stream) {
    if (!src || !index || !dst || n <= 0 || n_src_rows <= 0 || row_floats <= 0 || row_floats % 4 != 0 ||
        ((uintptr_t)src % 16) != 0 || ((uintptr_t)dst % 16) != 0)
        return PP_EINVAL;
    const long long n4 = row_floats / 4;
    const int gx = (int)((n4 + 255) / 256 < 64 ? (n4 + 255) / 256 : 64);
    hipLaunchKernelGGL(gather_rows_kernel, dim3(gx, n), dim3(256), 0, (hipStream_t)stream, src, index, row_floats, n_src_rows,
                       dst);
    return pp_last_launch();
}

int pp_bank_rows_to_tokens(const float* bank, long long n_bank_rows, int C, int P, const long long* index, int n, float* tokens, int ld,
                           int T, int skip, void* stream) {
    if (!bank || !index || !tokens || n_bank_rows <= 0 || C <= 0 || P <= 0 || n <= 0 || ld < C || skip < 0 || T <= 0 ||
        (long long)skip + P > T)
        return PP_EINVAL;
    if (n > 65535 || (P + 31) / 32 > 65535) return PP_EINVAL;
    hipLaunchKernelGGL(bank_rows_to_tokens_kernel, dim3((C + 31) / 32, (P + 31) / 32, n), dim3(256), 0, (hipStream_t)stream, bank, index,
                       n_bank_rows, C, P, tokens, ld, T, skip);
    return pp_last_launch();
}

int pp_saturation_take(unsigned int* word, unsigned int* slot, void* stream) {
    if (!word || !slot) return PP_EINVAL;
    hipLaunchKernelGGL(saturation_take_kernel, dim3(1), dim3(64), 0, (hipStream_t)stream, word, slot);
    return pp_last_launch();
}

int pp_crop_resize_normalize(const unsigned char* image, int H, int W, const unsigned char* mask, int y1, int y2, int x1,
                             int x2, int S, int rgb_mask_flag, const double* mean3, const double* std3, float* out_rgb,
                             float* out_mask, void* stream) {
    if (!image || !out_rgb || !mean3 || !std3 || H <= 0 || W <= 0 || S <= 0 || y1 < 0 || x1 < 0 || y2 > H || x2 > W ||
        y2 <= y1 || x2 <= x1)
        return PP_EINVAL;
    hipLaunchKernelGGL(crop_resize_kernel, dim3((S * S + 255) / 256), dim3(256), 0, (hipStream_t)stream, image, W, mask, y1, y2,
                       x1, x2, S, rgb_mask_flag, mean3[0], mean3[1], mean3[2], std3[0], std3[1], std3[2], out_rgb, out_mask);
    return pp_last_launch();
}

int pp_depth_points_nearest(const float* depth_m, int H, int W, int y1, int y2, int x1, int x2, int P, float fx, float fy,
                            float cx, float cy, float* out_pts, void* stream) {
    if (!depth_m || !out_pts || H <= 0 || W <= 0 || P <= 0 || y1 < 0 || x1 < 0 || y2 > H || x2 > W || y2 <= y1 || x2 <= x1 ||
        fx == 0.f || fy == 0.f)
        return PP_EINVAL;
    hipLaunchKernelGGL(depth_points_kernel, dim3((P * P + 255) / 256), dim3(256), 0, (hipStream_t)stream, depth_m, W, y1, y2, x1,
                       x2, P, fx, fy, cx, cy, out_pts);
    return pp_last_launch();
}

int pp_conv_narrow_hl(const void* x_hl, int ld_x, int B, int H, int W, int C, const float* weight, const float* bias, int ksize,
                      int n_out, const float* residual, float* out, void* stream) {
    if (!x_hl || !weight || !out || B <= 0 || H <= 0 || C <= 0 || C % 32 != 0 || ld_x < C || ld_x % 8 != 0) return PP_EINVAL;
    if ((W != 16 && W != 32 && W != 64) || H % (256 / W) != 0 || (ksize != 1 && ksize != 3) || (n_out != 1 && n_out != 2)) return PP_EINVAL;
    if (((uintptr_t)x_hl % 16) != 0) return PP_EINVAL;
    const int TH = 256 / W, R = ksize / 2;
    const size_t lds = (size_t)(TH + 2 * R) * (W + 2 * R) * NRW_PITCH;
    const dim3 grid((unsigned)(B * (H / TH)));
    hipStream_t st = (hipStream_t)stream;
#define NRW_LAUNCH(KS_, N_)                                                                                                        \
    hipLaunchKernelGGL((conv_narrow_kernel<KS_, N_>), grid, dim3(256), lds, st, (const _Float16*)x_hl, ld_x, H, W, C, weight, bias, \
                       residual, out)
    if (ksize == 3 && n_out == 2) NRW_LAUNCH(3, 2);
    else if (ksize == 3) NRW_LAUNCH(3, 1);
    else if (n_out == 2) NRW_LAUNCH(1, 2);
    else NRW_LAUNCH(1, 1);
#undef NRW_LAUNCH
    return pp_last_launch();
}

}
```

picopose_amd/model/stage1.py:

```python
import math

import torch
import torch.nn as nn
import torch.nn.functional as F

from .. import ops
from .common import Holder, Packed, conv_p, linear_p, norm_p

ARCH = {
    "vit_small": (384, 12, 6),
    "vit_base": (768, 12, 12),
    "vit_large": (1024, 24, 16),
    "vit_giant2": (1536, 40, 24),
}
DESCRIPTOR_MAP = {
    "dinov2_vits14": "vit_small",
    "dinov2_vitb14": "vit_base",
    "dinov2_vitl14": "vit_large",
    "dinov2_vitg14": "vit_giant2",
    "gigapose_dinov2": "vit_large",
}


def _block(dim):
# ... 12 lines not shown
    b.ls2.gamma = nn.Parameter(torch.ones(dim))
    return b


class DinoViT(Holder):
    def __init__(self, dim, depth, heads, img_size=518, patch=14):
        super().__init__()
        self.embed_dim = self.num_features = dim
        self.num_heads = heads
        self.patch_size = patch
        self.interpolate_offset = 0.1
        self.patch_embed = Holder()
        self.patch_embed.proj = conv_p(3, dim, patch)
        self.cls_token = nn.Parameter(torch.zeros(1, 1, dim))
        self.pos_embed = nn.Parameter(torch.zeros(1, (img_size // patch) ** 2 + 1, dim))
        self.blocks = nn.ModuleList([_block(dim) for _ in range(depth)])
        self.norm = norm_p(dim)
        self.mask_token = nn.Parameter(torch.zeros(1, dim))


class FeatureExtractor(Packed):
    def __init__(self, cfg, freeze=False):
        super().__init__()
        self.cfg = cfg
        self.blocks_to_take = [blocks[-1] for blocks in cfg.interaction_indexes]
        dim, depth, heads = ARCH[DESCRIPTOR_MAP[cfg.vit_type]]
        self.dinov2 = DinoViT(dim, depth, heads)
        self.num_features = dim
        self.patch_size = self.dinov2.patch_size

    def _pos_embed(self, w0, h0):
        v = self.dinov2
        pos = v.pos_embed.float()
        N = pos.shape[1] - 1
        if w0 * h0 == N:
            return pos[0]
        sq = int(math.sqrt(N))
        sx, sy = float(w0 + v.interpolate_offset) / math.sqrt(N), float(h0 + v.interpolate_offset) / math.sqrt(N)
        grid = F.interpolate(pos[:, 1:].reshape(1, sq, sq, -1).permute(0, 3, 1, 2), scale_factor=(sx, sy),
                             mode="bicubic", antialias=False)
        assert grid.shape[-2] == w0 and grid.shape[-1] == h0
        return torch.cat([pos[0, :1], grid.permute(0, 2, 3, 1).reshape(w0 * h0, -1)], dim=0)

    def _pack(self):
        v = self.dinov2
        return {
            "patch_w": ops.pack_conv_weight(v.patch_embed.proj.weight.float(), cin_pad=8),
            "pos": {},
        }

    def _pos_wt(self, w0, h0):
        v = self.dinov2
        cache = self.__dict__.setdefault("_pos_wt_cache", {})
        key = (v.pos_embed.shape[1] - 1, w0, h0, str(v.pos_embed.device))
        pk = {"pos": cache}
        if key not in pk["pos"]:
            N = v.pos_embed.shape[1] - 1
            if w0 * h0 == N:
                pk["pos"][key] = None
            else:
                sq = int(math.sqrt(N))
                sx, sy = float(w0 + v.interpolate_offset) / math.sqrt(N), float(h0 + v.interpolate_offset) / math.sqrt(N)
                with torch.no_grad():
                    basis = torch.eye(N, dtype=torch.float32, device=v.pos_embed.device).reshape(1, N, sq, sq)
                    grid = F.interpolate(basis, scale_factor=(sx, sy), mode="bicubic", antialias=False)
                pk["pos"][key] = grid.reshape(N, w0 * h0).contiguous()
        return pk["pos"][key]

    def _pos(self, w0, h0):
        pk = self.packed()
        key = (w0, h0)
        if key not in pk["pos"]:
            with torch.no_grad():
                wt = self._pos_wt(w0, h0) if self.training else None
                if wt is not None:
                    pe = self.dinov2.pos_embed.float()[0]
                    pk["pos"][key] = torch.cat([pe[:1], wt.t() @ pe[1:]], dim=0).contiguous()
                else:
                    pk["pos"][key] = self._pos_embed(w0, h0).contiguous()
        return pk["pos"][key]

    def forward_tokens(self, x, last_block_fn=None, all_blocks=False, embed_fn=None, level_out=None, full_depth=None):
        v = self.dinov2
        B, _, H, W = x.shape
        p = v.patch_size
        assert H % p == 0 and W % p == 0
        h0, w0 = H // p, W // p
        C, heads = v.embed_dim, v.num_heads
        hd = C // heads
        pk = self.packed()
        T = h0 * w0 + 1
        if embed_fn is not None:
            xs = embed_fn(self, x)
        else:
            img = ops.to_nhwc(x, c_pad=8)
            patches = ops.conv2d(img, pk["patch_w"], v.patch_embed.proj.bias, p, stride=p)
            tok = ops.assemble_tokens(patches.view(B, h0 * w0, C), v.cls_token.reshape(C), self._pos(h0, w0))
            xs = tok.view(B * T, C)
        outs = []
        if full_depth is not None:
            assert last_block_fn is None and embed_fn is None, "full_depth is an inference shortcut: not under the training hooks"
            assert len(self.blocks_to_take) >= 2 and 0 <= full_depth <= B
        for i, blk in enumerate(v.blocks):
            if full_depth is not None and i == self.blocks_to_take[-2] + 1:
                xs, B = xs[:full_depth * T], full_depth
                if B == 0:
                    outs.append(xs.view(0, T, C))
                    break
            if last_block_fn is not None and (all_blocks or i == len(v.blocks) - 1):
                xs = last_block_fn(blk, xs, B, T, heads, hd)
                if i in self.blocks_to_take:
                    outs.append(xs.view(B, T, C))
                continue
            h = ops.layernorm(xs, blk.norm1.weight, blk.norm1.bias, 1e-6, out_split=True)
            qkv = ops.linear(h, blk.attn.qkv.weight, blk.attn.qkv.bias, out_split=True)
            o = ops.attention(qkv, B, T, heads, hd, out_split=True)
            xs = ops.linear(o, blk.attn.proj.weight, blk.attn.proj.bias, gamma=blk.ls1.gamma, residual=xs)
            h = ops.layernorm(xs, blk.norm2.weight, blk.norm2.bias, 1e-6, out_split=True)
            f = ops.linear(h, blk.mlp.fc1.weight, blk.mlp.fc1.bias, act="gelu", out_split=True)
            dst = None
            if level_out is not None and i in self.blocks_to_take:
                dst = level_out[0][self.blocks_to_take.index(i)][level_out[1] * T:(level_out[1] + B) * T]
            xs = ops.linear(f, blk.mlp.fc2.weight, blk.mlp.fc2.bias, gamma=blk.ls2.gamma, residual=xs, out=dst)
            if i in self.blocks_to_take:
                outs.append(xs.view(B, T, C))
        return outs, (h0, w0)

    def forward(self, x):
        with torch.no_grad():
            toks, (h0, w0) = self.forward_tokens(x)
            return [ops.tokens_to_nchw(t, 1, h0, w0) for t in toks]
```

picopose_amd/model/stage3.py:

```python
import os

import torch
import torch.nn as nn

from .. import ops
from .common import Holder, Packed, bn_p, conv_p, convT_p, fold_bn, seq


COMPUTE_DEAD_LAYER1 = os.environ.get("PP_DPT_DEAD_LAYER1", "0") == "1"
OUT_CONV_FIRST = os.environ.get("PP_DPT_OUT_CONV_FIRST", "1") != "0"


def _rcu(c):
    m = Holder()
    m.conv1, m.conv2 = conv_p(c, c, 3), conv_p(c, c, 3)
    m.bn1, m.bn2 = bn_p(c), bn_p(c)
    return m


def _fusion(c):
    m = Holder()
    m.out_conv = conv_p(c, c, 1)
    m.resConfUnit1, m.resConfUnit2 = _rcu(c), _rcu(c)
    return m


class DPTHead(Packed):
    def __init__(self, nclass, in_channels, features=256, use_bn=False, out_channels=(256, 512, 1024, 1024),
                 use_clstoken=False):
        super().__init__()
        oc = list(out_channels)
        self.projects = nn.ModuleList([conv_p(in_channels, c, 1) for c in oc])
        self.resize_layers = seq((0, convT_p(oc[0], oc[0], 4)), (1, convT_p(oc[1], oc[1], 2)), (3, conv_p(oc[3], oc[3], 3)))
        s = Holder()
        for i in range(4):
            setattr(s, f"layer{i + 1}_rn", conv_p(oc[i], features, 3, bias=False))
        for i in range(4):
            setattr(s, f"refinenet{i + 1}", _fusion(features))
        s.output_conv1 = conv_p(features, features // 2, 3)
        s.output_conv2 = seq((0, conv_p(features // 2, 32, 3)), (2, conv_p(32, 1, 1)))
        self.scratch = s

    def _pack(self):
        pk = {}
        for i, p in enumerate(self.projects):
            pk[f"proj{i}"] = ops.pack_conv_weight(p.weight.float())
        r = self.resize_layers
        pk["up0"], pk["up0_b"] = ops.pack_convT_weight(getattr(r, "0").weight.float(), getattr(r, "0").bias.float())
        pk["up1"], pk["up1_b"] = ops.pack_convT_weight(getattr(r, "1").weight.float(), getattr(r, "1").bias.float())
        pk["down3"] = ops.pack_conv_weight(getattr(r, "3").weight.float())
        for i in range(4):
            pk[f"rn{i + 1}"] = ops.pack_conv_weight(getattr(self.scratch, f"layer{i + 1}_rn").weight.float())
        for i in (2, 3, 4):
            f = getattr(self.scratch, f"refinenet{i}")
            pk[f"f{i}_out"] = ops.pack_conv_weight(f.out_conv.weight.float())
            for j in (1, 2):
                u = getattr(f, f"resConfUnit{j}")
                for c in (1, 2):
                    w, b = fold_bn(getattr(u, f"conv{c}").weight.float(), getattr(u, f"conv{c}").bias.float(),
                                   getattr(u, f"bn{c}"))
                    pk[f"f{i}_u{j}_c{c}"], pk[f"f{i}_u{j}_b{c}"] = ops.pack_conv_weight(w), b.contiguous()
        return pk

    def _pack_train(self):
        pk = {}
        for i in (2, 3, 4):
            f = getattr(self.scratch, f"refinenet{i}")
            for j in (1, 2):
                u = getattr(f, f"resConfUnit{j}")
                for c in (1, 2):
                    pk[f"f{i}_u{j}_c{c}"] = ops.pack_conv_weight(getattr(u, f"conv{c}").weight.float())
        return pk

    def _rcu_train(self, i, j, x, extra=None):
        u, pkt = getattr(getattr(self.scratch, f"refinenet{i}"), f"resConfUnit{j}"), self.packed_train()
        h = ops.conv2d(x, pkt[f"f{i}_u{j}_c1"], u.conv1.bias, 3, pad=1, relu_in=True)
        h = ops.batchnorm_train(h, u.bn1, relu=True)
        h = ops.conv2d(h, pkt[f"f{i}_u{j}_c2"], u.conv2.bias, 3, pad=1)
        return ops.batchnorm_train(h, u.bn2, residual=x, residual2=extra)

    def _rcu(self, pk, key, x, extra=None, more=False, operand_only=False):
        xin = getattr(x, "_hl_relu", None)
        h = ops.conv2d(x if xin is None else xin, pk[key + "_c1"], pk[key + "_b1"], 3, pad=1, relu_in=xin is None,
                       out_split=True, split_relu=True, wino_next="relu")
        return ops.conv2d(h, pk[key + "_c2"], pk[key + "_b2"], 3, pad=1, relu_in=not isinstance(h, (ops.Split, ops.WinoInput)), residual=x,
                          residual2=extra, also_split="relu" if more else None, out_split=operand_only)

    def _fuse(self, pk, i, size, x0, x1=None, train=False):
        if train:
            out = x0 if x1 is None else self._rcu_train(i, 1, x1, extra=x0)
            out = self._rcu_train(i, 2, out)
        else:
            out = x0 if x1 is None else self._rcu(pk, f"f{i}_u1", x1, extra=x0, more=True)
            if OUT_CONV_FIRST:
                out = self._rcu(pk, f"f{i}_u2", out, operand_only=True)
                out = ops.conv2d(out, pk[f"f{i}_out"], getattr(self.scratch, f"refinenet{i}").out_conv.bias, 1)
                return ops.resize_bilinear(out, size[0], size[1], also_split=True)
            out = self._rcu(pk, f"f{i}_u2", out)
        out = ops.resize_bilinear(out, size[0], size[1], out_split=True)
        return ops.conv2d(out, pk[f"f{i}_out"], getattr(self.scratch, f"refinenet{i}").out_conv.bias, 1, also_split="plain")

    def forward_nhwc(self, feats, train=False):
        pk, r = self.packed(for_training=train), self.resize_layers
        live = range(4) if COMPUTE_DEAD_LAYER1 else range(1, 4)
        x = {i: ops.conv2d(feats[i], pk[f"proj{i}"], self.projects[i].bias, 1, out_split=True) for i in live}
        _, H0, W0, _ = feats[0].shape
        size1 = (4 * H0, 4 * W0)
        l2 = ops.conv_transpose2d(x[1], pk["up1"], pk["up1_b"], 2, out_split=True)
        l3 = x[2]
        l4 = ops.conv2d(x[3], pk["down3"], getattr(r, "3").bias, 3, stride=2, pad=1, out_split=True)
        rn = {i: ops.conv2d(l, pk[f"rn{i + 1}"], None, 3, pad=1, also_split="relu", wino=i in (1, 2)) for i, l in ((1, l2), (2, l3), (3, l4))}
        if COMPUTE_DEAD_LAYER1:
            l1 = ops.conv_transpose2d(x[0], pk["up0"], pk["up0_b"], 4, out_split=True)
            rn[0] = ops.conv2d(l1, pk["rn1"], None, 3, pad=1, also_split="relu")
            assert tuple(rn[0].shape[1:3]) == size1
        p4 = self._fuse(pk, 4, rn[2].shape[1:3], rn[3], train=train)
        p3 = self._fuse(pk, 3, rn[1].shape[1:3], p4, rn[2], train)
        p2 = self._fuse(pk, 2, size1, p3, rn[1], train)
        if train:
            self.bn_moved()
        return [p4, p3, p2]

    def forward(self, out_features):
        with torch.no_grad():
            return [ops.to_nchw(p) for p in self.forward_nhwc([ops.to_nhwc(f) for f in out_features])]


def _cm(cin, cout, k):
    m = Holder()
    m.conv = conv_p(cin, cout, k)
    return m


def _motion_encoder(levels, radius):
    m = Holder()
    m.corr_net = seq((0, _cm(levels * (2 * radius + 1) ** 2, 256, 1)), (1, _cm(256, 192, 3)))
    m.flow_net = seq((0, _cm(2, 128, 7)), (1, _cm(128, 64, 3)))
    m.out_net = seq((0, _cm(256, 126, 3)))
    return m


FUSE_XHEADS = os.environ.get("PP_FUSE_XHEADS", "0") == "1"


def _xhead(cin, kind):
    m = Holder()
    m.layers = seq((0, _cm(cin, 512, 3)), (1, _cm(512, 256, 3)))
    m.predict_layer = conv_p(256, 2, 3) if kind == "flow" else conv_p(256, 1, 1)
    return m


class FlowDecoder(Packed):
    def __init__(self, num_levels, radius):
        super().__init__()
        self.num_levels, self.radius = num_levels, radius
        self.r = int(radius / 2)
        self.proj = nn.ModuleList([seq((0, conv_p(256, 256, 1)), (1, bn_p(256))) for _ in range(num_levels)])
        self.encoder = nn.ModuleList([_motion_encoder(l + 1, self.r) for l in range(num_levels)])
        self.flow_pred = nn.ModuleList([_xhead(640, "flow") for _ in range(num_levels)])
        self.mask_pred = nn.ModuleList([_xhead(640, "mask") for _ in range(num_levels)])

    def _pack(self):
        pk = {}
        for l in range(self.num_levels):
            w, b = fold_bn(getattr(self.proj[l], "0").weight.float(), getattr(self.proj[l], "0").bias.float(),
                           getattr(self.proj[l], "1"))
            pk[f"proj{l}"], pk[f"proj{l}_b"] = ops.pack_conv_weight(w), b.contiguous()
            e = self.encoder[l]
            for name, net in (("corr", e.corr_net), ("flow", e.flow_net), ("out", e.out_net)):
                for idx, sub in net.named_children():
                    w = sub.conv.weight.float()
                    pad = -(-w.shape[1] // 8) * 8 if w.shape[1] % 8 else None
                    pk[f"e{l}_{name}{idx}"] = ops.pack_conv_weight(w, cin_pad=pad)
            w126 = pk[f"e{l}_out0"]
            pk[f"e{l}_out0_128"] = torch.cat([w126, w126.new_zeros(2, w126.shape[1])]).contiguous()
            b126 = getattr(e.out_net, "0").conv.bias.float()
            pk[f"e{l}_out0_b128"] = torch.cat([b126, b126.new_zeros(2)]).contiguous()
            for name, head in (("fp", self.flow_pred[l]), ("mp", self.mask_pred[l])):
                for idx, sub in head.layers.named_children():
                    pk[f"{name}{l}_{idx}"] = ops.pack_conv_weight(sub.conv.weight.float())
                pk[f"{name}{l}_p"] = ops.pack_conv_weight(head.predict_layer.weight.float())
            pk[f"x{l}_0"] = torch.cat([pk[f"fp{l}_0"], pk[f"mp{l}_0"]]).contiguous()
            pk[f"x{l}_0_b"] = torch.cat([getattr(self.flow_pred[l].layers, "0").conv.bias.float(),
                                         getattr(self.mask_pred[l].layers, "0").conv.bias.float()]).contiguous()
        return pk

    def _pack_train(self):
        return {f"proj{l}": ops.pack_conv_weight(getattr(self.proj[l], "0").weight.float()) for l in range(self.num_levels)}

    def forward_nhwc(self, feat_render_list, feat_real_list, flow, cert, train=False):
        pkt = self.packed_train() if train else None
        pk = self.packed(for_training=train)
        flows, certs = [], []
        for l in range(self.num_levels):
            fr_in, fq_in = feat_render_list[l], feat_real_list[l]
            B, H, W, _ = fr_in.shape
            opcat = ops.presplit()
            dev = fr_in.device
            if opcat:
                Xs = ops.Split.empty(B * H * W, 640, dev)
                Xs.image = (B, H, W)
                X = None
            else:
                X = torch.empty(B, H, W, 640, dtype=torch.float32, device=dev)
            e = self.encoder[l]
            fr_src = getattr(fr_in, "_hl", fr_in)
            if train:
                pj = self.proj[l]
                fr = ops.batchnorm_train(ops.conv2d(fr_src, pkt[f"proj{l}"], getattr(pj, "0").bias, 1), getattr(pj, "1"))
                fq = ops.batchnorm_train(ops.conv2d(getattr(fq_in, "_hl", fq_in), pkt[f"proj{l}"], getattr(pj, "0").bias, 1), getattr(pj, "1"))
                if opcat:
                    ops.split_activation(fr, B, H * W, 256, H * W * 256, 256, into=(Xs, 0))
                else:
                    X[..., 0:256] = fr
            else:
                fq = ops.conv2d(getattr(fq_in, "_hl", fq_in), pk[f"proj{l}"], pk[f"proj{l}_b"], 1, also_split="plain" if opcat else None)
                if opcat:
                    fr = ops.conv2d(fr_src, pk[f"proj{l}"], pk[f"proj{l}_b"], 1, hl_into=(Xs, 0),
                                    out=torch.empty(B, H, W, 256, dtype=torch.float32, device=dev))
                else:
                    fr = ops.conv2d(fr_src, pk[f"proj{l}"], pk[f"proj{l}_b"], 1, out=X[..., 0:256])
            ncorr = (l + 1) * (2 * self.r + 1) ** 2
            hl_maps = dict(f1_hl=(Xs, 0), f2_hl=getattr(fq, "_hl", None)) if opcat and not train and ops.terms() == 2 else {}
            corr = ops.corr_lookup(fr, fq, flow, l + 1, self.r, c_pad=-(-ncorr // 8) * 8, **hl_maps)
            hl_cat = opcat
            if hl_cat:
                cf = ops.Split.empty(B * H * W, 256, dev)
                cf.image = (B, H, W)
            else:
                cf = torch.empty(B, H, W, 256, dtype=torch.float32, device=dev)
            c1 = ops.conv2d(corr, pk[f"e{l}_corr0"], getattr(e.corr_net, "0").conv.bias, 1, act="relu", out_split=True)
            ops.conv2d(c1, pk[f"e{l}_corr1"], getattr(e.corr_net, "1").conv.bias, 3, pad=1, act="relu",
                       **(dict(hl_into=(cf, 0)) if hl_cat else dict(out=cf[..., 0:192])))
            flow8 = torch.zeros(B, H, W, 8, dtype=torch.float32, device=dev)
            flow8[..., 0:2] = flow
            f1 = ops.conv2d(flow8, pk[f"e{l}_flow0"], getattr(e.flow_net, "0").conv.bias, 7, pad=3, act="relu", out_split=True)
            ops.conv2d(f1, pk[f"e{l}_flow1"], getattr(e.flow_net, "1").conv.bias, 3, pad=1, act="relu",
                       **(dict(hl_into=(cf, 192)) if hl_cat else dict(out=cf[..., 192:256])))
            if opcat:
                ops.conv2d(cf, pk[f"e{l}_out0_128"], pk[f"e{l}_out0_b128"], 3, pad=1, act="relu", hl_into=(Xs, 512))
                ops.hl_patch_columns(flow[..., 0:2].contiguous() if flow.shape[-1] != 2 else flow, Xs, 638)
                ops.warp(fq, flow, hl_into=(Xs, 256))
            else:
                ops.conv2d(cf, pk[f"e{l}_out0"], getattr(e.out_net, "0").conv.bias, 3, pad=1, act="relu", out=X[..., 512:638])
                X[..., 638:640] = flow
                ops.warp(fq, flow, out=X[..., 256:512])
                Xs = ops.split_image(X)
            fp, mp = self.flow_pred[l], self.mask_pred[l]
            if FUSE_XHEADS and isinstance(Xs, ops.Split) and B * H * W * 1024 * 2 * Xs.terms < 0xFFFFFF00:
                hx = ops.conv2d(Xs, pk[f"x{l}_0"], pk[f"x{l}_0_b"], 3, pad=1, act="relu", out_split=True)
                h = ops.conv2d(hx, pk[f"fp{l}_1"], getattr(fp.layers, "1").conv.bias, 3, pad=1, act="relu", out_split=True, in_cols=(0, 512))
                flow = ops.conv2d(h, pk[f"fp{l}_p"], fp.predict_layer.bias, 3, pad=1, residual=flow)
                h = ops.conv2d(hx, pk[f"mp{l}_1"], getattr(mp.layers, "1").conv.bias, 3, pad=1, act="relu", out_split=True, in_cols=(512, 512))
                cert = ops.conv2d(h, pk[f"mp{l}_p"], mp.predict_layer.bias, 1, residual=cert)
            else:
                Xs = ops.winograd_shared(Xs, cout=512)
                if isinstance(Xs, ops.WinoInput4):
                    hf, hm = ops.conv2d_wino_pair(Xs, (pk[f"fp{l}_0"], getattr(fp.layers, "0").conv.bias), (pk[f"mp{l}_0"], getattr(mp.layers, "0").conv.bias),
                                                  act="relu", out_split=True, wino_next=True)
                else:
                    hf = ops.conv2d(Xs, pk[f"fp{l}_0"], getattr(fp.layers, "0").conv.bias, 3, pad=1, act="relu", out_split=True, wino=True, wino_next=True)
                    hm = ops.conv2d(Xs, pk[f"mp{l}_0"], getattr(mp.layers, "0").conv.bias, 3, pad=1, act="relu", out_split=True, wino=True, wino_next=True)
                h = ops.conv2d(hf, pk[f"fp{l}_1"], getattr(fp.layers, "1").conv.bias, 3, pad=1, act="relu", out_split=True, wino=True)
                flow = ops.conv2d(h, pk[f"fp{l}_p"], fp.predict_layer.bias, 3, pad=1, residual=flow)
                h = ops.conv2d(hm, pk[f"mp{l}_1"], getattr(mp.layers, "1").conv.bias, 3, pad=1, act="relu", out_split=True, wino=True)
                cert = ops.conv2d(h, pk[f"mp{l}_p"], mp.predict_layer.bias, 1, residual=cert)
            flows.append(flow)
            certs.append(cert)
            if l != self.num_levels - 1:
                flow = ops.resize_bilinear(flow, 2 * H, 2 * W, mul=2.0)
                cert = ops.resize_bilinear(cert, 2 * H, 2 * W)
        if train:
            self.bn_moved()
        return flows, certs

    def forward(self, feat_render_list, feat_real_list, init_flow, init_certainty, iters=1):
        assert iters == 1
        with torch.no_grad():
            fl, ce = self.forward_nhwc([ops.to_nhwc(f) for f in feat_render_list], [ops.to_nhwc(f) for f in feat_real_list],
                                       ops.to_nhwc(init_flow), ops.to_nhwc(init_certainty))
            return [ops.to_nchw(f) for f in fl], [ops.to_nchw(c) for c in ce]


class OffsetRegressor(nn.Module):
    def __init__(self, cfg):
        super().__init__()
        self.dpt_head = DPTHead(cfg.nclass, cfg.in_channels, features=256, use_bn=True,
                                out_channels=[256, 512, 1024, 1024], use_clstoken=False)
        self.flow_decoder = FlowDecoder(cfg.num_levels, cfg.radius)

    def forward_nhwc(self, feats_tem, feats_real, init_flow, init_cert, train=False):
        tem = self.dpt_head.forward_nhwc(feats_tem, train)
        real = self.dpt_head.forward_nhwc(feats_real, train)
        return self.flow_decoder.forward_nhwc(tem, real, init_flow, init_cert, train)

    def forward(self, features_tem, features_real, init_flow, init_certainty):
        return self.flow_decoder(self.dpt_head(features_tem), self.dpt_head(features_real), init_flow, init_certainty)
```

picopose_amd/ops.py:

```python
import contextlib
import ctypes
import os
import threading

import torch

from . import _lib
from ._lib import PpGemmDesc

ACT = {None: 0, "none": 0, "relu": 1, "gelu": 2, "leaky01": 3, "tanh": 4}

PRECISION = "f16x3"
_PREC = {"f32": 0, "f16x3": 1, "f16": 2}
_split_cache = {}
_scope = threading.local()


def precision():
    return getattr(_scope, "mode", None) or PRECISION


def check_precision(mode):
    if mode is not None and mode not in _PREC:
        raise ValueError(f"unknown arithmetic mode {mode!r}: expected None or one of {sorted(_PREC)}")
# ... 150 lines not shown

def split_weight_tracked(w, owner, tag=""):
    import weakref

    key = (id(owner), tag)
    ent = _tracked_scale.get(key)
    if ent is None or ent[2]() is not owner:
        hl, scale = split_weight(w, cache=False)
        if len(_tracked_scale) > 8192:
            _tracked_scale.clear()
        _tracked_scale[key] = [scale, None, weakref.ref(owner)]
        return hl, scale
    if ent[1] is not None and ent[1][1].query():
        v = float(ent[1][0][0])
        if v > 0.0 and v == v and v != float("inf"):
            ent[0] = v
        ent[1] = None
    t = terms()
    hl = torch.empty(w.shape[0], t * w.shape[1], dtype=torch.float16, device=w.device)
    sdev = torch.full((1,), ent[0], dtype=torch.float32, device=w.device)
    _lib.check(_lib.lib().pp_split_with_scale_t(_p(w), w.numel(), t, _p(sdev), _p(hl), _lib.stream_ptr()), "pp_split_with_scale_t")
    if ent[1] is None:
        s2 = torch.empty(2, dtype=torch.float32, device=w.device)
        _lib.check(_lib.lib().pp_pow2_scale(_p(w), w.numel(), _p(s2), _lib.stream_ptr()), "pp_pow2_scale")
        host = torch.empty(2, dtype=torch.float32, pin_memory=True)
        host.copy_(s2, non_blocking=True)
        ev = torch.cuda.Event()
        ev.record()
        ent[1] = (host, ev)
    return hl, ent[0]


class Split:
    __slots__ = ("hl", "image", "terms")

    def __init__(self, hl, t=None):
        self.hl = hl
        self.image = None
        self.terms = t or terms()

    @property
    def shape(self):
        return torch.Size((self.hl.shape[0], self.hl.shape[1] // self.terms))

    @property
    def device(self):
        return self.hl.device

    @staticmethod
    def empty(rows, C, device):
        return Split(torch.empty(rows, terms() * C, dtype=torch.float16, device=device))

    def cols(self, col0, c):
        return self.hl[:, self.terms * col0:self.terms * (col0 + c)]

    def col_ptr(self, col0):
        return self.hl.data_ptr() + 2 * self.terms * col0


def _split_ok(C):
    return presplit() and C % 8 == 0


def split_activation(x, B, P, C, batch_stride, row_stride, relu=False, into=None):
    t = terms()
    if into is not None:
        tgt, col0 = into
        ctot = tgt.shape[1]
        assert tgt.shape[0] == B * P and col0 % 8 == 0 and col0 + C <= ctot
        _lib.check(_lib.lib().pp_split_activation_t(_p(x), batch_stride, B, P, row_stride, C, int(relu),
                                                    tgt.col_ptr(col0), ctot, t, _lib.stream_ptr()), "pp_split_activation_t")
        if CHECK_SATURATION:
            _chk(tgt.cols(col0, C), "pp_split_activation_t")
        return None
    hl = torch.empty(B * P, t * C, dtype=torch.float16, device=x.device)
    _lib.check(_lib.lib().pp_split_activation_t(_p(x), batch_stride, B, P, row_stride, C, int(relu), _p(hl), C, t,
                                                _lib.stream_ptr()), "pp_split_activation_t")
    return _chk(hl, "pp_split_activation_t")


def hl_patch_columns(x, tgt, col0):
    c = x.shape[-1]
    rows = x.numel() // c
    assert x.is_contiguous() and rows == tgt.shape[0] and col0 + c <= tgt.shape[1]
    _lib.check(_lib.lib().pp_hl_patch_columns_t(_p(x), c, c, rows, _p(tgt.hl), tgt.shape[1], col0, tgt.terms, _lib.stream_ptr()),
               "pp_hl_patch_columns_t")
    if CHECK_SATURATION:
        _chk(tgt.cols(col0 // 8 * 8, -(-(col0 + c) // 8) * 8 - col0 // 8 * 8), "pp_hl_patch_columns_t")


def _can_presplit(x, K, C, *strides):
    return (presplit() and K % 8 == 0 and C % 8 == 0 and x.data_ptr() % 16 == 0
            and all(st % 4 == 0 for st in strides))


def _weight_args(w, K, cache=True):
    if isinstance(cache, tuple) and os.environ.get("PP_TRACK_SCALE", "1") == "0":
        cache = False
    if presplit() and K % 8 == 0 and w.data_ptr() % 16 == 0:
        if cache == "dev":
            hl, s2 = split_weight_dev(w)
            return dict(prec=_PREC[precision()], B_hl=_p(hl), b_scale=1.0, alpha_dev=_p(s2[1:2]), _hl=(hl, s2))
        hl, scale = split_weight_tracked(w, *cache) if isinstance(cache, tuple) else split_weight(w, cache)
        return dict(prec=_PREC[precision()], B_hl=_p(hl), b_scale=scale, _hl=hl)
    return dict(prec=_fly_prec())


def _fly_prec():
    return 0 if precision() == "f32" else 1


def _fly_args(wargs, w=None, cache=True):
    if precision() == "f16":
        if w is not None and cache is True and "B_hl" in wargs:
            hl, scale = split_weight(w, True, t=2)
            return dict(prec=1, B_hl=_p(hl), b_scale=scale, _hl=hl)
        return dict(prec=1)
    if "alpha_dev" in wargs:
        return dict(prec=_fly_prec())
    return wargs


def _p(t):
    return t.data_ptr() if t is not None else None


def _run(d, what="pp_gemm", written=None):
    _lib.check(_lib.lib().pp_gemm(ctypes.byref(d), _lib.stream_ptr()), what)
    if written is not None:
        _chk(written.hl, f"{what} epilogue (M={d.M}, N={d.N}, K={d.K})")


def _desc(**kw):
    d = PpGemmDesc()
    d.batch0 = d.batch1 = 1
    d.alpha = 1.0
    for k, v in kw.items():
        if not k.startswith("_"):
            setattr(d, k, v)
    return d


def linear(x, weight, bias=None, act=None, gamma=None, residual=None, out=None, relu_in=False, out_split=False, cache_weight=True):
    M, K = x.shape
    N = weight.shape[0]
    assert weight.shape[1] == K and weight.is_contiguous()
    wargs = _weight_args(weight, K, cache_weight)
    sargs, ret = {}, None
    if out_split and "B_hl" in wargs and _split_ok(N) and out is None:
        ret = Split.empty(M, N, x.device)
        sargs = dict(C_hl=_p(ret.hl), ldc_h=N)
    elif out is None:
        out = torch.empty(M, N, dtype=torch.float32, device=x.device)
    ldc = N if out is None else out.stride(0)
    if out is not None:
        assert out.stride(1) == 1
        ret = out
    if residual is not None:
        assert tuple(residual.shape) == (M, N) and residual.stride(1) == 1 and residual.stride(0) == ldc
    if isinstance(x, Split):
        assert "B_hl" in wargs
        _run(_desc(A_hl=_p(x.hl), B=_p(weight), C=_p(out), bias=_p(bias), gamma=_p(gamma), residual=_p(residual),
                   M=M, N=N, K=K, lda=K, ldb=K, ldc=ldc, act=ACT[act], **wargs, **sargs), written=ret if sargs else None)
        return ret
    assert x.stride(1) == 1
    if "B_hl" in wargs and N > 64 and _can_presplit(x, K, K, x.stride(0)) and M * K < 2 ** 31:
        hl = split_activation(x, 1, M, K, 0, x.stride(0), relu=relu_in)
        _run(_desc(A_hl=_p(hl), B=_p(weight), C=_p(out), bias=_p(bias), gamma=_p(gamma), residual=_p(residual),
                   M=M, N=N, K=K, lda=K, ldb=K, ldc=ldc, act=ACT[act], **wargs, **sargs), written=ret if sargs else None)
        return ret
    if sargs:
# ... 597 lines not shown
    for r in (residual, residual2):
        assert r is None or (r.is_contiguous() and r.shape == x.shape)
    _lib.check(L.pp_batchnorm_train(_p(x), _p(bn.weight), _p(bn.bias), rows, C, float(eps), float(momentum), _p(bn.running_mean),
                                    _p(bn.running_var), int(relu), _p(residual) if residual is not None else None,
                                    _p(residual2) if residual2 is not None else None, _p(y), _p(ws), nbytes, _lib.stream_ptr()),
               "pp_batchnorm_train")
    bn.num_batches_tracked += 1
    return y


def to_nhwc(x, c_pad=None):
    B, C, H, W = x.shape
    x = x.contiguous().float()
    Cp = c_pad if c_pad and c_pad > C else C
    out = (torch.zeros if Cp > C else torch.empty)(B, H, W, Cp, dtype=torch.float32, device=x.device)
    _lib.check(_lib.lib().pp_transpose_batched(_p(x), 0, B, C, H * W, _p(out), 0, Cp, 0, _lib.stream_ptr()),
               "pp_transpose_batched")
    return out


def to_nchw(x):
    B, H, W, C = x.shape
    assert x.is_contiguous()
    out = torch.empty(B, C, H, W, dtype=torch.float32, device=x.device)
    _lib.check(_lib.lib().pp_transpose_batched(_p(x), 0, B, H * W, C, _p(out), 0, H * W, 0, _lib.stream_ptr()),
               "pp_transpose_batched")
    return out


def resize_bilinear(x, Ho, Wo, mul=1.0, out_split=False, also_split=False):
    B, H, W, C = x.shape
    assert x.is_contiguous()
    if also_split and _split_ok(C) and x.data_ptr() % 16 == 0:
        out = torch.empty(B, Ho, Wo, C, dtype=torch.float32, device=x.device)
        sp = Split.empty(B * Ho * Wo, C, x.device)
        sp.image = (B, Ho, Wo)
        _lib.check(_lib.lib().pp_resize_bilinear_nhwc_dual(_p(x), B, H, W, C, Ho, Wo, float(mul), _p(out), _p(sp.hl), sp.terms,
                                                            _lib.stream_ptr()), "pp_resize_bilinear_nhwc_dual")
        _chk(sp.hl, "pp_resize_bilinear_nhwc_dual")
        out._hl = sp
        return out
    if out_split and _split_ok(C) and x.data_ptr() % 16 == 0:
        sp = Split.empty(B * Ho * Wo, C, x.device)
        sp.image = (B, Ho, Wo)
        _lib.check(_lib.lib().pp_resize_bilinear_nhwc_t(_p(x), B, H, W, C, Ho, Wo, float(mul), _p(sp.hl), sp.terms, _lib.stream_ptr()),
                   "pp_resize_bilinear_nhwc_t")
        _chk(sp.hl, "pp_resize_bilinear_nhwc_t")
        return sp
    out = torch.empty(B, Ho, Wo, C, dtype=torch.float32, device=x.device)
    _lib.check(_lib.lib().pp_resize_bilinear_nhwc(_p(x), B, H, W, C, Ho, Wo, float(mul), _p(out), _lib.stream_ptr()),
               "pp_resize_bilinear_nhwc")
    return out


def warp(feat, flow, out=None, hl_into=None):
    B, H, W = flow.shape[:3]
    Bf, Hf, Wf, C = feat.shape
    assert (Hf, Wf) == (H, W) and B % Bf == 0
    assert feat.is_contiguous() and flow.stride(3) == 1 and flow.stride(2) * W == flow.stride(1)
    if hl_into is not None:
        tgt, col0 = hl_into
        ctot = tgt.shape[1]
        assert tgt.shape[0] == B * H * W and col0 % 8 == 0 and col0 + C <= ctot and C % 8 == 0
        _lib.check(_lib.lib().pp_warp_nhwc_t(_p(feat), Bf, _p(flow), B, H, W, C, flow.stride(2), tgt.col_ptr(col0),
                                             ctot, tgt.terms, _lib.stream_ptr()), "pp_warp_nhwc_t")
        if CHECK_SATURATION:
            _chk(tgt.cols(col0, C), "pp_warp_nhwc_t")
        return None
    if out is None:
        out = torch.empty(B, H, W, C, dtype=torch.float32, device=feat.device)
    _lib.check(_lib.lib().pp_warp_nhwc(_p(feat), Bf, _p(flow), B, H, W, C, flow.stride(2), _p(out), out.stride(2),
                                       _lib.stream_ptr()), "pp_warp_nhwc")
    return out


def avgpool2(x):
    B, H, W, C = x.shape
    assert x.is_contiguous()
    out = torch.empty(B, H // 2, W // 2, C, dtype=torch.float32, device=x.device)
    _lib.check(_lib.lib().pp_avgpool2_nhwc(_p(x), B, H, W, C, _p(out), _lib.stream_ptr()), "pp_avgpool2_nhwc")
    return out


def corr_lookup(f1, f2, flow, levels, radius, c_pad=None, f1_hl=None, f2_hl=None):
    B, H, W, C = f1.shape
    assert f2.is_contiguous() and flow.stride(3) == 1 and B % f2.shape[0] == 0 and tuple(f2.shape[1:]) == (H, W, C)
    assert f1.stride(3) == 1 and f1.stride(1) == W * f1.stride(2) and f1.stride(0) == H * f1.stride(1)
    pyr = [f2]
    for _ in range(levels - 1):
        pyr.append(avgpool2(pyr[-1]))
    n = levels * (2 * radius + 1) ** 2
    np_ = c_pad if c_pad and c_pad > n else n
    out = (torch.zeros if np_ > n else torch.empty)(B, H, W, np_, dtype=torch.float32, device=f1.device)
    if (f1_hl is not None and f2_hl is not None and precision() == "f16x3" and f2_hl.terms == 2 and H % 8 == 0 and W % 8 == 0 and C % 32 == 0
            and os.environ.get("PP_CORR_TILED", "1") != "0" and os.environ.get("PP_CORR_HL", "1") != "0"):
        tgt, col0 = f1_hl
        assert tgt.shape[0] == B * H * W and col0 % 8 == 0 and col0 + C <= tgt.shape[1] and f2_hl.shape == (f2.shape[0] * H * W, C)
        hls = [f2_hl.hl] + [split_activation(p, p.shape[0], p.shape[1] * p.shape[2], C, p.shape[1] * p.shape[2] * C, C) for p in pyr[1:]]
        _lib.check(_lib.lib().pp_corr_lookup_nhwc_hl(tgt.hl.data_ptr() + 4 * col0, tgt.shape[1], _p(hls[0]), _p(hls[1]) if levels > 1 else None,
                                                     _p(hls[2]) if levels > 2 else None, f2.shape[0], _p(flow), B, H, W, C, levels, radius,
                                                     flow.stride(2), _p(out), np_, _lib.stream_ptr()), "pp_corr_lookup_nhwc_hl")
        return out
    _lib.check(_lib.lib().pp_corr_lookup_nhwc_ex(_p(f1), f1.stride(2), _p(pyr[0]), _p(pyr[1]) if levels > 1 else None,
                                                 _p(pyr[2]) if levels > 2 else None, f2.shape[0], _p(flow), B, H, W, C,
                                                 levels, radius, flow.stride(2), 2 if precision() == "f16" else _fly_prec(), _p(out), np_,
                                                 _lib.stream_ptr()), "pp_corr_lookup_nhwc_ex")
    return out


def tokens_to_nchw(tokens, skip, H, W):
    B, T, C = tokens.shape
    assert tokens.is_contiguous()
    out = torch.empty(B, C, H, W, dtype=torch.float32, device=tokens.device)
    src = tokens[:, skip:]
    _lib.check(_lib.lib().pp_transpose_batched(_p(src), T * C, B, H * W, C, _p(out), 0, H * W, 0, _lib.stream_ptr()),
               "pp_transpose_batched")
    return out


def assemble_tokens(patches, cls_token, pos):
    B, T, C = patches.shape
    assert patches.is_contiguous() and pos.is_contiguous() and cls_token.is_contiguous()
    out = torch.empty(B, T + 1, C, dtype=torch.float32, device=patches.device)
    _lib.check(_lib.lib().pp_assemble_tokens(_p(patches), _p(cls_token), _p(pos), B, T, C, _p(out), _lib.stream_ptr()),
               "pp_assemble_tokens")
    return out


def normalize_rows(x, eps=1e-12):
    rows, n = x.shape
    assert x.is_contiguous()
    y = torch.empty_like(x)
    _lib.check(_lib.lib().pp_normalize_rows(_p(x), rows, n, float(eps), _p(y), _lib.stream_ptr()), "pp_normalize_rows")
    return y


def gather_rows(src, index):
    R = src.shape[0]
    row = src[0].numel()
    if row % 4 != 0 or not src.is_contiguous() or src.dtype != torch.float32 or src.data_ptr() % 16 != 0:
        return src[index]
    index = index.contiguous()
    dst = torch.empty((index.numel(),) + tuple(src.shape[1:]), dtype=torch.float32, device=src.device)
    _lib.check(_lib.lib().pp_gather_rows(_p(src), _p(index), R, row, index.numel(), _p(dst), _lib.stream_ptr()),
               "pp_gather_rows")
    return dst


def bank_rows_to_tokens(bank, index, T, skip=1, out=None):
    R, C = bank.shape[:2]
    P = bank[0, 0].numel()
    n = index.numel()
    assert bank.is_contiguous() and bank.dtype == torch.float32 and index.dtype == torch.int64 and index.device == bank.device
    if out is None:
        out = torch.empty(n * T, C, dtype=torch.float32, device=bank.device)
    assert out.dim() == 2 and out.dtype == torch.float32 and out.shape[0] == n * T and out.shape[1] >= C and out.stride(1) == 1 and out.device == bank.device
    _lib.check(_lib.lib().pp_bank_rows_to_tokens(_p(bank), R, C, P, _p(index.contiguous()), n, _p(out), out.stride(0), T, skip,
                                                 _lib.stream_ptr()), "pp_bank_rows_to_tokens")
    return out
```

picopose_amd/picopose.py:

```python
import os

import torch
import torch.nn as nn

from . import ops
from .model.stage1 import FeatureExtractor
from .model.stage2 import AffineRegressor
from .model.stage3 import OffsetRegressor
from .utils.augment import aug_gtM_noise
from .utils.correspondence import compute_init_correspondences, compute_stage3_correspondences
from .utils.keypoints import KeypointInput, KeyPointSampler
from .utils.loss_utils import compute_stage_two_loss, flow_level_losses, infonce_rows
from .utils.matching import matching_features_similarity, matching_templates, matching_templates_indexed
from .utils.pose_recovery import pose_recovery_2d_prediction
from .utils.torch_utils import calc_pred_Ms


BATCH_VIT_TRAIN = os.environ.get("PP_BATCH_VIT_TRAIN", "1") != "0"
BATCH_DPT = os.environ.get("PP_BATCH_DPT", "1") != "0"
PREFETCH_QUERY = os.environ.get("PP_PREFETCH_QUERY", "1") != "0"
TEMPLATE_LAST_FROM_BANK = {"0": False, "1": True}.get(os.environ.get("PP_TEMPLATE_LAST_FROM_BANK"))


def _tensor_key(t, fe=None):
    key = (t.data_ptr(), tuple(t.shape), t._version, ops.precision())
    return key if fe is None else key + (fe._signatures()[0],)


def _image_rows(p, b0, b1):
    q = p[b0:b1]
    hl = getattr(p, "_hl", None)
    if hl is not None:
        hw = p.shape[1] * p.shape[2]
        s = ops.Split(hl.hl[b0 * hw:b1 * hw], hl.terms)
        s.image = (b1 - b0, p.shape[1], p.shape[2])
        q._hl = s
    return q


class Net(nn.Module):
    def __init__(self, cfg):
        super().__init__()
        self.cfg = cfg
        self.keypoint_sampler = KeyPointSampler()
        self.feature_extractor = FeatureExtractor(cfg.stage1)
        self.affine_regressor = AffineRegressor(cfg.stage2)
        self.offset_regressor = OffsetRegressor(cfg.stage3)
        self.match_mode = None
        self.batch_hypotheses = True
        self.keep_stage3 = False
        self.last_stage3 = None
        self.train_backward = True
        self.precision = None
        self.template_last_from_bank = None
        self.range_fallbacks = 0

    @property
    def precision(self):
        return self._precision

    @precision.setter
    def precision(self, mode):
        self._precision = ops.check_precision(mode)

    def invalidate_packed(self):
        from .model.common import Packed

        for m in self.modules():
            if isinstance(m, Packed):
                m.invalidate_packed()
        self._query_stash = None

    def _last_from_bank(self, end_points):
        on = self.template_last_from_bank
        on = TEMPLATE_LAST_FROM_BANK if on is None else on
        on = ops.precision() in ("f16x3", "f16") if on is None else on
        bank = end_points.get("template_feature")
        if not on or self.training or bank is None or end_points.get("template_cache") is not None:
            return False
        fe = self.feature_extractor
        H, W = end_points["tem_rgb"].shape[-2:]
        grid = (fe.num_features, H // fe.patch_size, W // fe.patch_size)
        return (bank.dtype == torch.float32 and bank.dim() == 5 and tuple(bank.shape[2:]) == grid and bank.is_contiguous()
                and tuple(bank.shape[:2]) == tuple(end_points["tem_rgb"].shape[:2]) and len(fe.blocks_to_take) >= 2)

    def select_template_data(self, end_points, pred_id_src, k):
        idx = pred_id_src[:, k]
        rows = end_points.get("template_index")
        rows = torch.arange(idx.shape[0], device=idx.device) if rows is None else rows
        sel = {key: end_points[key][rows, idx] for key in ("tem_pose", "tem_K", "tem_M", "tem_mask", "tem_rgb", "tem_pts3d")}
        if self._last_from_bank(end_points):
            sel["tem_bank"] = (end_points["template_feature"].flatten(0, 1), rows * end_points["template_feature"].shape[1] + idx)
        for key in ("real_pts2d", "real_K", "real_M", "real_mask", "real_pose"):
            sel[key] = end_points[key]
        return sel

    def precompute_templates(self, tem_rgb, chunk=54):
        fe, dpt = self.feature_extractor, self.offset_regressor.dpt_head
        feats, maps = [], [[], [], []]
        with torch.no_grad():
            for s0 in range(0, tem_rgb.shape[0], chunk):
                toks, (h0, w0) = fe.forward_tokens(tem_rgb[s0:s0 + chunk])
                feats.append(ops.tokens_to_nchw(toks[-1], 1, h0, w0))
                for k, m in enumerate(dpt.forward_nhwc([t[:, 1:].unflatten(1, (h0, w0)) for t in toks])):
                    maps[k].append(m)
        return {"feature": torch.cat(feats), "dpt": [torch.cat(m) for m in maps]}

    def forward_test_hyp(self, end_points, real, tem_cached=None):
        fe = self.feature_extractor
        real_tok, (h0, w0) = real[0], real[1]
        real_dpt = real[2] if len(real) > 2 else None
        levels = real[3] if len(real) > 3 else None
        output = {"tem_pose": end_points["tem_pose"]}
        output["tar_pts_2d"] = end_points["real_pts2d"].permute(0, 3, 2, 1)
        output["src_pts_3d"] = end_points["tem_pts3d"].permute(0, 3, 1, 2)
        pre = real[4] if len(real) > 4 else None
        bank = end_points.get("tem_bank") if tem_cached is None else None
        T = h0 * w0 + 1
        if tem_cached is None and pre is not None and levels is not None:
            alloc, nxt = pre
            Bn = nxt.shape[0]
            both, _ = fe.forward_tokens(torch.cat([nxt, end_points["tem_rgb"]]), level_out=(alloc, 0), full_depth=None if bank is None else Bn)
            tem_tok = [t[Bn:] for t in both]
            if bank is not None:
                nT = tem_tok[0].shape[0]
                tem_tok[-1] = ops.bank_rows_to_tokens(*bank, T, out=alloc[-1][Bn * T:(Bn + nT) * T]).view(nT, T, -1)
            self._query_stash = (_tensor_key(nxt, fe), [a[:Bn * T].clone() for a in alloc], (h0, w0), nxt)
        elif tem_cached is None:
            tem_tok, _ = fe.forward_tokens(end_points["tem_rgb"], level_out=None if levels is None else (levels, 0),
                                           full_depth=None if bank is None else 0)
            if bank is not None:
                nT = tem_tok[0].shape[0]
                tem_tok[-1] = ops.bank_rows_to_tokens(*bank, T, out=None if levels is None else levels[-1][:nT * T]).view(nT, T, -1)
        else:
            tem_last, tem_dpt = tem_cached
        if tem_cached is None:
            tem_last = ops.tokens_to_nchw(tem_tok[-1], 1, h0, w0) if bank is None else ops.gather_rows(*bank)
        sim = matching_features_similarity(tem_last, ops.tokens_to_nchw(real_tok[-1], 1, h0, w0),
                                           end_points["tem_mask"], end_points["real_mask"])
        pred_translation, pred_scale, pred_inplane = self.affine_regressor(sim)
        pred_Ms = calc_pred_Ms(pred_scale, pred_inplane, pred_translation, end_points["tem_pose"], end_points["tem_K"],
                               end_points["tem_M"])
        output["pred_poses"] = pose_recovery_2d_prediction(end_points["real_M"], end_points["real_K"], pred_Ms,
                                                           end_points["tem_K"], end_points["tem_M"], end_points["tem_pose"])
        init_flow, init_certainty = compute_init_correspondences(pred_Ms, end_points["tem_mask"])
        as_img = lambda t: t[:, 1:].unflatten(1, (h0, w0))
        orr = self.offset_regressor
        if levels is not None and real_dpt is None and tem_cached is None:
            nT, nR = tem_tok[0].shape[0], levels[0].shape[0] // T - tem_tok[0].shape[0]
            both = orr.dpt_head.forward_nhwc([as_img(lv.view(-1, T, lv.shape[1])) for lv in levels])
            tem_dpt, real_dpt = [_image_rows(p_, 0, nT) for p_ in both], [_image_rows(p_, nT, nT + nR) for p_ in both]
        else:
            if real_dpt is None:
                real_dpt = orr.dpt_head.forward_nhwc([as_img(t) for t in real_tok])
            if tem_cached is None:
                tem_dpt = orr.dpt_head.forward_nhwc([as_img(t) for t in tem_tok])
        flows, certs = orr.flow_decoder.forward_nhwc(tem_dpt, real_dpt, ops.to_nhwc(init_flow), ops.to_nhwc(init_certainty))
        if self.keep_stage3:
            self.last_stage3 = (flows[-1], certs[-1])
        output["pred_tar_pts"], output["pred_src_pts"] = compute_stage3_correspondences(
            ops.to_nchw(flows[-1]), ops.to_nchw(certs[-1]), threshold=0.5)
        return output

    def forward_hypotheses(self, end_points, pred_id_src, real):
        hyp = pred_id_src.shape[1]
        cache = end_points.get("template_cache")
        tidx = end_points.get("template_index")

        def cached(rows, idx):
            if cache is None:
                return None
            obj = (cache["obj_index"] if tidx is None else tidx)[rows]
            return end_points["template_feature"][rows if tidx is None else obj, idx], [m[obj, idx] for m in cache["dpt"]]

        if not self.batch_hypotheses:
            rows = torch.arange(pred_id_src.shape[0], device=pred_id_src.device)
            return [self.forward_test_hyp(self.select_template_data(end_points, pred_id_src, k), real,
                                          cached(rows, pred_id_src[:, k])) for k in range(hyp)]
        real_tok, hw = real[0], real[1]
        real_dpt = real[2] if len(real) > 2 and real[2] is not None else None
        levels = real[3] if len(real) > 3 else None
        B = pred_id_src.shape[0]
        idx = pred_id_src.t().reshape(-1)
        rows = torch.arange(B, device=idx.device).repeat(hyp)
        rep = lambda t: t.repeat(hyp, *([1] * (t.dim() - 1)))
        N = end_points["tem_pose"].shape[1]
        trow = rows if tidx is None else tidx[rows]
        flat = trow * N + idx
        sel = {key: (ops.gather_rows(end_points[key].flatten(0, 1), flat) if end_points[key].is_contiguous()
                     else end_points[key][trow, idx])
               for key in ("tem_pose", "tem_K", "tem_M", "tem_mask", "tem_rgb", "tem_pts3d")}
        if self._last_from_bank(end_points):
            sel["tem_bank"] = (end_points["template_feature"].flatten(0, 1), flat)
        for key in ("real_pts2d", "real_K", "real_M", "real_mask", "real_pose"):
            sel[key] = rep(end_points[key])
        toks = ([rep(t) for t in real_tok] if real_dpt is None and levels is None
                else [None] * (len(real_tok) - 1) + [rep(real_tok[-1])])
        out = self.forward_test_hyp(sel, (toks, hw, real_dpt, levels if cache is None else None, real[4] if len(real) > 4 and cache is None else None),
                                    cached(rows, idx))
        return [{key: v[k * B:(k + 1) * B] for key, v in out.items()} for k in range(hyp)]

    TEMPLATE_KEYS = ("template_feature", "tem_pose", "tem_K", "tem_M", "tem_mask", "tem_rgb", "tem_pts3d")

    def _check_template_index(self, end_points):
        tidx = end_points["template_index"]
        B = end_points["real_rgb"].shape[0]
        if not isinstance(tidx, torch.Tensor) or tidx.dtype != torch.int64 or tuple(tidx.shape) != (B,) or tidx.device != end_points["real_rgb"].device:
            raise ValueError(f"template_index must be a ({B},) int64 tensor on the crops' device")
        lead = {key: tuple(end_points[key].shape[:2]) for key in self.TEMPLATE_KEYS if key in end_points}
        if len(set(lead.values())) != 1:
            raise ValueError(f"with template_index every template tensor is (O, N, ...) for the same O and N: {lead}")
        cache = end_points.get("template_cache")
        if cache is not None and cache["obj_index"] is not tidx and not torch.equal(cache["obj_index"].to(tidx.device), tidx):
            raise ValueError("template_cache['obj_index'] and template_index name different objects")

    def forward_test(self, end_points, hyp=5, next_real_rgb=None):
        with torch.no_grad():
            if "template_index" in end_points:
                self._check_template_index(end_points)
            fe = self.feature_extractor
            levels = None
            ops.saturation_word(end_points["real_rgb"].device)
            stash, self._query_stash = getattr(self, "_query_stash", None), None
            if BATCH_DPT and self.batch_hypotheses and end_points.get("template_cache") is None:
                B, _, H, W = end_points["real_rgb"].shape
                T = (H // fe.patch_size) * (W // fe.patch_size) + 1
                pre_ok = PREFETCH_QUERY and next_real_rgb is not None and tuple(next_real_rgb.shape[1:]) == (3, H, W) and next_real_rgb.is_contiguous()
                Bn = next_real_rgb.shape[0] if pre_ok else 0
                alloc = [torch.empty((Bn + (hyp + 1) * B) * T, fe.num_features, dtype=torch.float32, device=end_points["real_rgb"].device)
                         for _ in fe.blocks_to_take]
                levels = [a_[Bn * T:] for a_ in alloc]
                if stash is not None and stash[0] == _tensor_key(end_points["real_rgb"], fe) and stash[1][0].shape[0] == B * T:
                    (h0, w0) = stash[2]
                    for lv, st in zip(levels, stash[1]):
                        lv[hyp * B * T:].copy_(st)
                    real_tok = [lv[hyp * B * T:].view(B, T, -1) for lv in levels]
                else:
                    real_tok, (h0, w0) = fe.forward_tokens(end_points["real_rgb"], level_out=(levels, hyp * B))
                real = (real_tok, (h0, w0), None, levels, (alloc, next_real_rgb) if Bn else None)
            else:
                real_tok, (h0, w0) = fe.forward_tokens(end_points["real_rgb"])
                real_dpt = self.offset_regressor.dpt_head.forward_nhwc([t[:, 1:].unflatten(1, (h0, w0)) for t in real_tok])
                real = (real_tok, (h0, w0), real_dpt)
            query = ops.tokens_to_nchw(real_tok[-1], 1, h0, w0)
            if "template_index" in end_points:
                pred_score_src, pred_id_src = matching_templates_indexed(
                    end_points["template_feature"], end_points["template_index"], query, end_points["tem_mask"], end_points["real_mask"],
                    topk=hyp, mode=self.match_mode)
            else:
                pred_score_src, pred_id_src = matching_templates(
                    end_points["template_feature"], query, end_points["tem_mask"], end_points["real_mask"], topk=hyp, mode=self.match_mode)
            return self.forward_hypotheses(end_points, pred_id_src, real)

    def compute_keypoint_data(self, end_points):
        rel_pose = end_points["tem_pose"] @ torch.inverse(end_points["real_pose"])
        tar = KeypointInput(full_depth=end_points["real_full_depth"], K=end_points["real_K"], M=end_points["real_M"], mask=end_points["real_mask"])
        src = KeypointInput(full_depth=end_points["tem_full_depth"], K=end_points["tem_K"], M=end_points["tem_M"], mask=end_points["tem_mask"])
        return self.keypoint_sampler.sample_pts(tar_data=tar, src_data=src, T_src2target=torch.inverse(rel_pose), T_tar2source=rel_pose)

    def forward_train(self, end_points, pred_Ms=None):
        from . import autograd as ag
        from .utils.loss_utils import infonce_index_rows

        live = torch.is_grad_enabled() and bool(self.train_backward)
        wide = live and self.train_backward != "slice1"
        full = wide and self.train_backward != "vit+stage2"
        fe, orr = self.feature_extractor, self.offset_regressor
        with torch.no_grad():
            kp = self.compute_keypoint_data(end_points)
        with torch.set_grad_enabled(live):
            kw = dict(last_block_fn=ag.last_block_forward if live else None, all_blocks=wide, embed_fn=ag.embed_tokens if wide else None)
            if BATCH_VIT_TRAIN and end_points["real_rgb"].shape == end_points["tem_rgb"].shape:
                nb = end_points["real_rgb"].shape[0]
                both, (h0, w0) = fe.forward_tokens(torch.cat([end_points["real_rgb"], end_points["tem_rgb"]]), **kw)
# ... 53 lines not shown
```

Before: 568.3.

## Build split-f16 operands directly from bank rows and flow; skip dead fp32 maps

A new kernel gathers template RGB rows from the bank and writes them straight into the split f16 hi/lo operand layout, replacing a gather, a concat and an NHWC conversion before patch embedding. A second kernel builds the flow operand directly. A lean decoder mode lets the correlation lookup run from operand-form maps only, so the fp32 projection output and the finest DPT fp32 output are never materialised, and zero-fill of padded outputs moves into the kernels. A 256x192 GEMM tile is also added for N sizes that leave a 128-192 remainder. Together these cut memory traffic and launches, at the cost of added code paths and shape conditions.

```diff
diff --git a/include/picopose_hip.h b/include/picopose_hip.h
--- a/include/picopose_hip.h
+++ b/include/picopose_hip.h
@@ -203,6 +203,9 @@
                    void* stream);
 int pp_bank_rows_to_tokens(const float* bank, long long n_bank_rows, int C, int P, const long long* index, int n, float* tokens, int ld,
                            int T, int skip, void* stream);
+int pp_patch_operand(const float* bank, long long n_bank_rows, const long long* index, int n, const float* front, int n_front, int H, int W,
+                     void* out, int terms, void* stream);
+int pp_flow_operand(const float* flow, int ld_flow, long long rows, void* out8, int terms, void* stream);
 
 int pp_crop_resize_normalize(const unsigned char* image, int H, int W, const unsigned char* mask, int y1, int y2, int x1,
                              int x2, int S, int rgb_mask_flag, const double* mean3, const double* std3, float* out_rgb,
diff --git a/picopose_amd/_lib.py b/picopose_amd/_lib.py
--- a/picopose_amd/_lib.py
+++ b/picopose_amd/_lib.py
@@ -150,6 +150,8 @@
         L.pp_avgpool2_nhwc.argtypes = [vp, i32, i32, i32, i32, vp, vp]
         L.pp_gather_rows.argtypes = [vp, vp, c.c_longlong, c.c_longlong, i32, vp, vp]
         L.pp_bank_rows_to_tokens.argtypes = [vp, c.c_longlong, i32, i32, vp, i32, vp, i32, i32, i32, vp]
+        L.pp_patch_operand.argtypes = [vp, c.c_longlong, vp, i32, vp, i32, i32, i32, vp, i32, vp]
+        L.pp_flow_operand.argtypes = [vp, i32, c.c_longlong, vp, i32, vp]
         L.pp_depth_points_nearest.argtypes = [vp, i32, i32, i32, i32, i32, i32, i32, f32, f32, f32, f32, vp, vp]
         L.pp_crop_resize_normalize.argtypes = [vp, i32, i32, vp, i32, i32, i32, i32, i32, i32, c.POINTER(c.c_double),
                                                c.POINTER(c.c_double), vp, vp, vp]
diff --git a/picopose_amd/csrc/pp_gemm.hip b/picopose_amd/csrc/pp_gemm.hip
--- a/picopose_amd/csrc/pp_gemm.hip
+++ b/picopose_amd/csrc/pp_gemm.hip
@@ -1174,8 +1174,9 @@
         if (cfg == 5 && d.N <= 128) cfg = 4;
         if (!v.u_vec && cfg != 2) cfg = 0;
         p.engine = cfg == 6 ? GE_UH : GE_U;
-        p.tile = cfg == 5 ? PP_U_256x256 : cfg == 4 ? PP_U_256x128 : cfg == 2 ? PP_U_128x64 : PP_U_128x128;
         p.amode = cfg == 6 ? 1 : pp_gemm_u_mode(d, v.terms);
+        if (cfg == 11 && p.amode == 3) cfg = 4;
+        p.tile = cfg == 11 ? PP_U_256x192 : cfg == 5 ? PP_U_256x256 : cfg == 4 ? PP_U_256x128 : cfg == 2 ? PP_U_128x64 : PP_U_128x128;
         p.vec = v.u_vec;
     } else if (v.fvec && (cfg >= 3 || d.grp_rows != 0)) {
         if (cfg < 3) cfg = 3;
@@ -1245,6 +1246,8 @@
         if (t4 >= cus / 2) c[n++] = 4;
         if (t5 >= cus / 2 && d.N > 128) c[n++] = 5;
         if (t5 >= cus / 2 && d.N > 128 && v.h_shape) c[n++] = 6;
+        static const bool tile192 = [] { const char* e = getenv("PP_GEMM_TILE_192"); return !(e && e[0] == '0'); }();
+        if (tile192 && d.N % 256 > 128 && d.N % 256 <= 192 && v.u_vec && (long long)((d.M + 255) / 256) * ((d.N + 191) / 192) >= cus / 2) c[n++] = 11;
         if (tail_on && d.N > 128 && tail_rows(v, 256, cus)) c[n++] = 9;
         if (tail_on && tail_rows(v, 128, cus)) c[n++] = 10;
     } else if (v.fvec) {
@@ -1314,7 +1317,7 @@
     bool pinned = false;
     if (const char* f = getenv("PP_GEMM_FORCE_CFG")) {
         const int fc = atoi(f);
-        if (((fc == 9 || fc == 10) && (v.asplit || v.fvec)) || (fc >= 0 && fc <= 8 && (v.asplit || fc <= 2 || (v.fvec && fc <= 7)))) {
+        if (((fc == 9 || fc == 10) && (v.asplit || v.fvec)) || (fc == 11 && v.asplit) || (fc >= 0 && fc <= 8 && (v.asplit || fc <= 2 || (v.fvec && fc <= 7)))) {
             cfg = fc;
             pinned = true;
         }
diff --git a/picopose_amd/csrc/pp_gemm_u.h b/picopose_amd/csrc/pp_gemm_u.h
--- a/picopose_amd/csrc/pp_gemm_u.h
+++ b/picopose_amd/csrc/pp_gemm_u.h
@@ -3,7 +3,8 @@
 #include <hip/hip_runtime.h>
 #include "../../include/picopose_hip.h"
 
-enum { PP_U_128x64 = 0, PP_U_128x128 = 1, PP_U_256x128 = 2, PP_U_256x256 = 3, PP_F_256x192 = 4  };
+enum { PP_U_128x64 = 0, PP_U_128x128 = 1, PP_U_256x128 = 2, PP_U_256x256 = 3, PP_F_256x192 = 4 ,
+       PP_U_256x192 = 5  };
 
 int pp_gemm_u_mode(const PpGemmDesc& d, int terms);
 int pp_gemm_u_launch_t1(const PpGemmDesc& d, int tile, int mode, bool vec, int cus, hipStream_t st);
diff --git a/picopose_amd/csrc/pp_gemm_u_kernel.h b/picopose_amd/csrc/pp_gemm_u_kernel.h
--- a/picopose_amd/csrc/pp_gemm_u_kernel.h
+++ b/picopose_amd/csrc/pp_gemm_u_kernel.h
@@ -864,6 +864,7 @@
 typedef TileCfg<256, 128, 4, 2, 3, 1, 1> T256x128;
 typedef TileCfg<128, 128, 2, 2, 2, 2> T128x128;
 typedef TileCfg<128, 64, 2, 2, 3, 2> T128x64;
+typedef TileCfg<256, 192, 4, 2, 2, 1> T256x192;
 
 template <class T, int MODE, int TERMS, bool VEC, int EPI = PP_EPI_GENERIC>
 static int pp_u_launch_one(const PpGemmDesc& d, int persistent_slots, hipStream_t st) {
@@ -895,7 +896,7 @@
     if (mode == 0) return pp_u_launch_one<T, 0, TERMS, VEC>(d, slots, st);
     if (mode == 1) return pp_u_launch_one<T, 1, TERMS, VEC>(d, slots, st);
     if (mode == 3) {
-        if constexpr (TERMS == 2 && VEC) return pp_u_launch_one<T, 3, TERMS, VEC>(d, slots, st);
+        if constexpr (TERMS == 2 && VEC && !std::is_same<T, T256x192>::value) return pp_u_launch_one<T, 3, TERMS, VEC>(d, slots, st);
         else return PP_EINVAL;
     }
     return pp_u_launch_one<T, 2, TERMS, VEC>(d, slots, st);
@@ -911,6 +912,7 @@
     switch (tile) {
         case PP_U_256x256: return pp_u_launch_tile<T256x256, TERMS, true>(d, mode, cus, st);
         case PP_U_256x128: return pp_u_launch_tile<T256x128, TERMS, true>(d, mode, cus, st);
+        case PP_U_256x192: return pp_u_launch_tile<T256x192, TERMS, true>(d, mode, cus, st);
         case PP_U_128x128: return pp_u_launch_tile<T128x128, TERMS, true>(d, mode, 2 * cus, st);
         case PP_U_128x64: return pp_u_launch_tile<T128x64, TERMS, true>(d, mode, 2 * cus, st);
         default: return PP_EINVAL;
diff --git a/picopose_amd/csrc/pp_sample.hip b/picopose_amd/csrc/pp_sample.hip
--- a/picopose_amd/csrc/pp_sample.hip
+++ b/picopose_amd/csrc/pp_sample.hip
@@ -227,6 +227,7 @@
             const float* t = tab + l * tw * tw + bi * tw + ai;
             o[i] = t[0] * (wx0 * wy0) + t[1] * (wx1 * wy0) + t[tw] * (wx0 * wy1) + t[tw + 1] * (wx1 * wy1);
         }
+        for (int i = nout + lane; i < ld_out; i += 64) o[i] = 0.f;
     }
 }
 
@@ -264,6 +265,10 @@
         gx = (float)(x0 + mx) + fl[0];
         gy = (float)(y0 + my) + fl[1];
     }
+    for (int npad = ld_out - L * win * win, idx = tid; idx < CM * npad; idx += 256) {
+        const int m = idx / npad, o = idx - m * npad;
+        out[((size_t)b * H * W + (size_t)(y0 + (m >> 3)) * W + x0 + (m & 7)) * ld_out + L * win * win + o] = 0.f;
+    }
     for (int l = 0; l < L; ++l) {
         const int Hl = H >> l, Wl = W >> l;
         const void* f2v = l == 0 ? f2l0 : (l == 1 ? f2l1 : f2l2);
@@ -604,6 +609,67 @@
         float v = (F32IN ? acc[n] : acc[n] * (1.0f / PP_A_SCALE)) + (bias ? bias[n] : 0.f);
         if (residual) v += residual[o + n];
         out[o + n] = v;
+    }
+}
+
+__global__ __launch_bounds__(256) void flow_operand_kernel(const float* __restrict__ flow, int ld_flow, long long rows, _Float16* __restrict__ op8,
+                                                           int terms) {
+    const long long p = (long long)blockIdx.x * 256 + threadIdx.x;
+    if (p >= rows) return;
+    const float* f = flow + p * ld_flow;
+    _Float16 h0, l0, h1, l1;
+    pp_split_f16_chk(f[0], h0, l0);
+    pp_split_f16_chk(f[1], h1, l1);
+    const _Float16 z = (_Float16)0.f;
+    const h8_t hi = {h0, h1, z, z, z, z, z, z}, lo = {l0, l1, z, z, z, z, z, z};
+    h8_t* o = (h8_t*)(op8 + p * 8 * terms);
+    o[0] = hi;
+    if (terms == 2) o[1] = lo;
+}
+
+constexpr int PO_TILE = 1024;
+__global__ __launch_bounds__(256) void patch_operand_kernel(const float* __restrict__ bank, const long long* __restrict__ index, long long n_rows,
+                                                            const float* __restrict__ front, int n_front, int HW, _Float16* __restrict__ out,
+                                                            int terms) {
+    __shared__ __attribute__((aligned(16))) float t[3][PO_TILE];
+    const int j = blockIdx.y, tid = threadIdx.x;
+    const float* src;
+    if (j < n_front) {
+        src = front + (size_t)j * 3 * HW;
+    } else {
+        const long long r = index[j - n_front];
+        if (r < 0 || r >= n_rows) return;
+        src = bank + (size_t)r * 3 * HW;
+    }
+    const int p0 = blockIdx.x * PO_TILE, np = min(PO_TILE, HW - p0);
+    if ((HW & 3) == 0) {
+        for (int i = tid; i < 3 * (np >> 2); i += 256) {
+            const int c = i / (np >> 2), q = i - c * (np >> 2);
+            *(f4*)&t[c][4 * q] = *(const f4*)(src + (size_t)c * HW + p0 + 4 * q);
+        }
+    } else {
+        for (int i = tid; i < 3 * np; i += 256) {
+            const int c = i / np, q = i - c * np;
+            t[c][q] = src[(size_t)c * HW + p0 + q];
+        }
+    }
+    __syncthreads();
+    h8_t* o = (h8_t*)(out + ((size_t)j * HW + p0) * 8 * terms);
+    const _Float16 z = (_Float16)0.f;
+    for (int i = tid; i < np * terms; i += 256) {
+        const int q = terms == 2 ? i >> 1 : i;
+        _Float16 h0, l0, h1, l1, h2, l2;
+        if (terms == 1 || (i & 1) == 0) {
+            pp_split_f16_chk(t[0][q], h0, l0);
+            pp_split_f16_chk(t[1][q], h1, l1);
+            pp_split_f16_chk(t[2][q], h2, l2);
+            o[i] = h8_t{h0, h1, h2, z, z, z, z, z};
+        } else {
+            pp_split_f16(t[0][q], h0, l0);
+            pp_split_f16(t[1][q], h1, l1);
+            pp_split_f16(t[2][q], h2, l2);
+            o[i] = h8_t{l0, l1, l2, z, z, z, z, z};
+        }
     }
 }
 
@@ -801,6 +867,26 @@
     return pp_last_launch();
 }
 
+int pp_patch_operand(const float* bank, long long n_bank_rows, const long long* index, int n, const float* front, int n_front, int H, int W,
+                     void* out, int terms, void* stream) {
+    if (!out || n < 0 || n_front < 0 || n + n_front <= 0 || H <= 0 || W <= 0 || (terms != 1 && terms != 2)) return PP_EINVAL;
+    if ((n > 0 && (!bank || !index || n_bank_rows <= 0)) || (n_front > 0 && !front)) return PP_EINVAL;
+    if (((uintptr_t)out | (n > 0 ? (uintptr_t)bank : 0) | (n_front > 0 ? (uintptr_t)front : 0)) % 16 != 0) return PP_EINVAL;
+    const long long hw = (long long)H * W, tiles = (hw + PO_TILE - 1) / PO_TILE;
+    if (n + n_front > 65535 || hw > 0x7fffffff || tiles > 0x7fffffff) return PP_EINVAL;
+    hipLaunchKernelGGL(patch_operand_kernel, dim3((unsigned)tiles, n + n_front), dim3(256), 0, (hipStream_t)stream, bank, index, n_bank_rows,
+                       front, n_front, (int)hw, (_Float16*)out, terms);
+    return pp_last_launch();
+}
+
+int pp_flow_operand(const float* flow, int ld_flow, long long rows, void* out8, int terms, void* stream) {
+    if (!flow || !out8 || rows <= 0 || ld_flow < 2 || ((uintptr_t)out8 % 16) != 0 || (terms != 1 && terms != 2)) return PP_EINVAL;
+    if ((rows + 255) / 256 > 0x7fffffff) return PP_EINVAL;
+    hipLaunchKernelGGL(flow_operand_kernel, dim3((unsigned)((rows + 255) / 256)), dim3(256), 0, (hipStream_t)stream, flow, ld_flow, rows,
+                       (_Float16*)out8, terms);
+    return pp_last_launch();
+}
+
 int pp_saturation_take(unsigned int* word, unsigned int* slot, void* stream) {
     if (!word || !slot) return PP_EINVAL;
     hipLaunchKernelGGL(saturation_take_kernel, dim3(1), dim3(64), 0, (hipStream_t)stream, word, slot);
diff --git a/picopose_amd/model/stage1.py b/picopose_amd/model/stage1.py
--- a/picopose_amd/model/stage1.py
+++ b/picopose_amd/model/stage1.py
@@ -118,7 +118,7 @@
 
     def forward_tokens(self, x, last_block_fn=None, all_blocks=False, embed_fn=None, level_out=None, full_depth=None):
         v = self.dinov2
-        B, _, H, W = x.shape
+        B, H, W = x.image if isinstance(x, ops.Split) else (x.shape[0],) + tuple(x.shape[2:])
         p = v.patch_size
         assert H % p == 0 and W % p == 0
         h0, w0 = H // p, W // p
@@ -129,7 +129,7 @@
         if embed_fn is not None:
             xs = embed_fn(self, x)
         else:
-            img = ops.to_nhwc(x, c_pad=8)
+            img = x if isinstance(x, ops.Split) else ops.to_nhwc(x, c_pad=8)
             patches = ops.conv2d(img, pk["patch_w"], v.patch_embed.proj.bias, p, stride=p)
             tok = ops.assemble_tokens(patches.view(B, h0 * w0, C), v.cls_token.reshape(C), self._pos(h0, w0))
             xs = tok.view(B * T, C)
diff --git a/picopose_amd/model/stage3.py b/picopose_amd/model/stage3.py
--- a/picopose_amd/model/stage3.py
+++ b/picopose_amd/model/stage3.py
@@ -86,7 +86,7 @@
         return ops.conv2d(h, pk[key + "_c2"], pk[key + "_b2"], 3, pad=1, relu_in=not isinstance(h, (ops.Split, ops.WinoInput)), residual=x,
                           residual2=extra, also_split="relu" if more else None, out_split=operand_only)
 
-    def _fuse(self, pk, i, size, x0, x1=None, train=False):
+    def _fuse(self, pk, i, size, x0, x1=None, train=False, operand_only=False):
         if train:
             out = x0 if x1 is None else self._rcu_train(i, 1, x1, extra=x0)
             out = self._rcu_train(i, 2, out)
@@ -95,12 +95,12 @@
             if OUT_CONV_FIRST:
                 out = self._rcu(pk, f"f{i}_u2", out, operand_only=True)
                 out = ops.conv2d(out, pk[f"f{i}_out"], getattr(self.scratch, f"refinenet{i}").out_conv.bias, 1)
-                return ops.resize_bilinear(out, size[0], size[1], also_split=True)
+                return ops.resize_bilinear(out, size[0], size[1], **(dict(out_split=True) if operand_only else dict(also_split=True)))
             out = self._rcu(pk, f"f{i}_u2", out)
         out = ops.resize_bilinear(out, size[0], size[1], out_split=True)
         return ops.conv2d(out, pk[f"f{i}_out"], getattr(self.scratch, f"refinenet{i}").out_conv.bias, 1, also_split="plain")
 
-    def forward_nhwc(self, feats, train=False):
+    def forward_nhwc(self, feats, train=False, finest_operand_only=False):
         pk, r = self.packed(for_training=train), self.resize_layers
         live = range(4) if COMPUTE_DEAD_LAYER1 else range(1, 4)
         x = {i: ops.conv2d(feats[i], pk[f"proj{i}"], self.projects[i].bias, 1, out_split=True) for i in live}
@@ -116,7 +116,7 @@
             assert tuple(rn[0].shape[1:3]) == size1
         p4 = self._fuse(pk, 4, rn[2].shape[1:3], rn[3], train=train)
         p3 = self._fuse(pk, 3, rn[1].shape[1:3], p4, rn[2], train)
-        p2 = self._fuse(pk, 2, size1, p3, rn[1], train)
+        p2 = self._fuse(pk, 2, size1, p3, rn[1], train, operand_only=finest_operand_only and not train and ops.decoder_lean())
         if train:
             self.bn_moved()
         return [p4, p3, p2]
@@ -192,9 +192,10 @@
         pkt = self.packed_train() if train else None
         pk = self.packed(for_training=train)
         flows, certs = [], []
+        lean = ops.decoder_lean() and not train
         for l in range(self.num_levels):
             fr_in, fq_in = feat_render_list[l], feat_real_list[l]
-            B, H, W, _ = fr_in.shape
+            B, H, W = fr_in.image if isinstance(fr_in, ops.Split) else fr_in.shape[:3]
             opcat = ops.presplit()
             dev = fr_in.device
             if opcat:
@@ -215,13 +216,14 @@
                     X[..., 0:256] = fr
             else:
                 fq = ops.conv2d(getattr(fq_in, "_hl", fq_in), pk[f"proj{l}"], pk[f"proj{l}_b"], 1, also_split="plain" if opcat else None)
-                if opcat:
-                    fr = ops.conv2d(fr_src, pk[f"proj{l}"], pk[f"proj{l}_b"], 1, hl_into=(Xs, 0),
-                                    out=torch.empty(B, H, W, 256, dtype=torch.float32, device=dev))
-                else:
-                    fr = ops.conv2d(fr_src, pk[f"proj{l}"], pk[f"proj{l}_b"], 1, out=X[..., 0:256])
+            hl_maps = dict(f1_hl=(Xs, 0), f2_hl=getattr(fq, "_hl", None)) if opcat and not train and ops.terms() == 2 else {}
+            if not train and opcat:
+                fr_dead = lean and bool(hl_maps) and ops.corr_takes_operands(hl_maps["f1_hl"], hl_maps["f2_hl"], H, W, 256)
+                fr = ops.conv2d(fr_src, pk[f"proj{l}"], pk[f"proj{l}_b"], 1, hl_into=(Xs, 0),
+                                out=None if fr_dead else torch.empty(B, H, W, 256, dtype=torch.float32, device=dev))
+            elif not train:
+                fr = ops.conv2d(fr_src, pk[f"proj{l}"], pk[f"proj{l}_b"], 1, out=X[..., 0:256])
             ncorr = (l + 1) * (2 * self.r + 1) ** 2
-            hl_maps = dict(f1_hl=(Xs, 0), f2_hl=getattr(fq, "_hl", None)) if opcat and not train and ops.terms() == 2 else {}
             corr = ops.corr_lookup(fr, fq, flow, l + 1, self.r, c_pad=-(-ncorr // 8) * 8, **hl_maps)
             hl_cat = opcat
             if hl_cat:
@@ -232,14 +234,17 @@
             c1 = ops.conv2d(corr, pk[f"e{l}_corr0"], getattr(e.corr_net, "0").conv.bias, 1, act="relu", out_split=True)
             ops.conv2d(c1, pk[f"e{l}_corr1"], getattr(e.corr_net, "1").conv.bias, 3, pad=1, act="relu",
                        **(dict(hl_into=(cf, 0)) if hl_cat else dict(out=cf[..., 0:192])))
-            flow8 = torch.zeros(B, H, W, 8, dtype=torch.float32, device=dev)
-            flow8[..., 0:2] = flow
-            f1 = ops.conv2d(flow8, pk[f"e{l}_flow0"], getattr(e.flow_net, "0").conv.bias, 7, pad=3, act="relu", out_split=True)
+            if lean and opcat:
+                flow8 = ops.flow_operand(flow)
+            else:
+                flow8 = torch.zeros(B, H, W, 8, dtype=torch.float32, device=dev)
+                flow8[..., 0:2] = flow
+            f1 =ops.conv2d(flow8, pk[f"e{l}_flow0"], getattr(e.flow_net, "0").conv.bias, 7, pad=3, act="relu", out_split=True)
             ops.conv2d(f1, pk[f"e{l}_flow1"], getattr(e.flow_net, "1").conv.bias, 3, pad=1, act="relu",
                        **(dict(hl_into=(cf, 192)) if hl_cat else dict(out=cf[..., 192:256])))
             if opcat:
                 ops.conv2d(cf, pk[f"e{l}_out0_128"], pk[f"e{l}_out0_b128"], 3, pad=1, act="relu", hl_into=(Xs, 512))
-                ops.hl_patch_columns(flow[..., 0:2].contiguous() if flow.shape[-1] != 2 else flow, Xs, 638)
+                ops.hl_patch_columns(flow[..., 0:2] if lean else (flow[..., 0:2].contiguous() if flow.shape[-1] != 2 else flow), Xs, 638)
                 ops.warp(fq, flow, hl_into=(Xs, 256))
             else:
                 ops.conv2d(cf, pk[f"e{l}_out0"], getattr(e.out_net, "0").conv.bias, 3, pad=1, act="relu", out=X[..., 512:638])
diff --git a/picopose_amd/ops.py b/picopose_amd/ops.py
--- a/picopose_amd/ops.py
+++ b/picopose_amd/ops.py
@@ -256,11 +256,47 @@
 def hl_patch_columns(x, tgt, col0):
     c = x.shape[-1]
     rows = x.numel() // c
-    assert x.is_contiguous() and rows == tgt.shape[0] and col0 + c <= tgt.shape[1]
-    _lib.check(_lib.lib().pp_hl_patch_columns_t(_p(x), c, c, rows, _p(tgt.hl), tgt.shape[1], col0, tgt.terms, _lib.stream_ptr()),
+    ld = c if x.is_contiguous() else x.stride(-2)
+    assert rows == tgt.shape[0] and col0 + c <= tgt.shape[1]
+    assert x.is_contiguous() or (x.dim() >= 2 and x.stride(-1) == 1 and ld >= c
+                                 and all(x.stride(i) == x.stride(i + 1) * x.shape[i + 1] for i in range(x.dim() - 2)))
+    _lib.check(_lib.lib().pp_hl_patch_columns_t(_p(x), ld, c, rows, _p(tgt.hl), tgt.shape[1], col0, tgt.terms, _lib.stream_ptr()),
                "pp_hl_patch_columns_t")
     if CHECK_SATURATION:
         _chk(tgt.cols(col0 // 8 * 8, -(-(col0 + c) // 8) * 8 - col0 // 8 * 8), "pp_hl_patch_columns_t")
+
+
+def flow_operand(flow):
+    B, H, W = flow.shape[:3]
+    assert presplit() and flow.dtype == torch.float32 and flow.shape[3] >= 2 and flow.stride(3) == 1
+    assert flow.stride(1) == W * flow.stride(2) and flow.stride(0) == H * flow.stride(1)
+    sp = Split.empty(B * H * W, 8, flow.device)
+    sp.image = (B, H, W)
+    _lib.check(_lib.lib().pp_flow_operand(_p(flow), flow.stride(2), B * H * W, _p(sp.hl), sp.terms, _lib.stream_ptr()), "pp_flow_operand")
+    _chk(sp.hl, "pp_flow_operand")
+    return sp
+
+
+def patch_operand_on():
+    return os.environ.get("PP_PATCH_OPERAND", "1") != "0"
+
+
+def patch_operand_ok(bank, front=None):
+    ok = lambda t: (t.dim() == 4 and t.shape[1] == 3 and t.dtype == torch.float32 and t.is_contiguous() and t.data_ptr() % 16 == 0)
+    return (presplit() and ok(bank) and bank.shape[0] > 0
+            and (front is None or (ok(front) and front.shape[2:] == bank.shape[2:] and front.device == bank.device)))
+
+
+def patch_operand(bank, index, front=None):
+    assert patch_operand_ok(bank, front) and index.dtype == torch.int64 and index.device == bank.device
+    R, _, H, W = bank.shape
+    n, nf = index.numel(), 0 if front is None else front.shape[0]
+    sp = Split.empty((nf + n) * H * W, 8, bank.device)
+    sp.image = (nf + n, H, W)
+    _lib.check(_lib.lib().pp_patch_operand(_p(bank), R, _p(index.contiguous()), n, _p(front), nf, H, W, _p(sp.hl), sp.terms,
+                                           _lib.stream_ptr()), "pp_patch_operand")
+    _chk(sp.hl, "pp_patch_operand")
+    return sp
 
 
 def _can_presplit(x, K, C, *strides):
@@ -1024,18 +1060,30 @@
     return out
 
 
+def decoder_lean():
+    return os.environ.get("PP_DECODER_LEAN", "1") != "0"
+
+
+def corr_takes_operands(f1_hl, f2_hl, H, W, C):
+    return (f1_hl is not None and f2_hl is not None and precision() == "f16x3" and f2_hl.terms == 2 and H % 8 == 0 and W % 8 == 0 and C % 32 == 0
+            and os.environ.get("PP_CORR_TILED", "1") != "0" and os.environ.get("PP_CORR_HL", "1") != "0")
+
+
 def corr_lookup(f1, f2, flow, levels, radius, c_pad=None, f1_hl=None, f2_hl=None):
-    B, H, W, C = f1.shape
-    assert f2.is_contiguous() and flow.stride(3) == 1 and B % f2.shape[0] == 0 and tuple(f2.shape[1:]) == (H, W, C)
-    assert f1.stride(3) == 1 and f1.stride(1) == W * f1.stride(2) and f1.stride(0) == H * f1.stride(1)
+    (H, W, C), B = f2.shape[1:], flow.shape[0]
+    assert f2.is_contiguous() and flow.stride(3) == 1 and B % f2.shape[0] == 0 and tuple(flow.shape[1:3]) == (H, W)
+    operands = corr_takes_operands(f1_hl, f2_hl, H, W, C)
+    if f1 is None:
+        assert operands, "corr_lookup without the fp32 map f1 needs the operand form of both maps (corr_takes_operands)"
+    else:
+        assert tuple(f1.shape) == (B, H, W, C) and f1.stride(3) == 1 and f1.stride(1) == W * f1.stride(2) and f1.stride(0) == H * f1.stride(1)
     pyr = [f2]
     for _ in range(levels - 1):
         pyr.append(avgpool2(pyr[-1]))
     n = levels * (2 * radius + 1) ** 2
     np_ = c_pad if c_pad and c_pad > n else n
-    out = (torch.zeros if np_ > n else torch.empty)(B, H, W, np_, dtype=torch.float32, device=f1.device)
-    if (f1_hl is not None and f2_hl is not None and precision() == "f16x3" and f2_hl.terms == 2 and H % 8 == 0 and W % 8 == 0 and C % 32 == 0
-            and os.environ.get("PP_CORR_TILED", "1") != "0" and os.environ.get("PP_CORR_HL", "1") != "0"):
+    out = (torch.zeros if np_ > n and not decoder_lean() else torch.empty)(B, H, W, np_, dtype=torch.float32, device=f2.device)
+    if operands:
         tgt, col0 = f1_hl
         assert tgt.shape[0] == B * H * W and col0 % 8 == 0 and col0 + C <= tgt.shape[1] and f2_hl.shape == (f2.shape[0] * H * W, C)
         hls = [f2_hl.hl] + [split_activation(p, p.shape[0], p.shape[1] * p.shape[2], C, p.shape[1] * p.shape[2] * C, C) for p in pyr[1:]]
diff --git a/picopose_amd/picopose.py b/picopose_amd/picopose.py
--- a/picopose_amd/picopose.py
+++ b/picopose_amd/picopose.py
@@ -28,6 +28,11 @@
 
 
 def _image_rows(p, b0, b1):
+    if isinstance(p, ops.Split):
+        hw = p.image[1] * p.image[2]
+        s = ops.Split(p.hl[b0 * hw:b1 * hw], p.terms)
+        s.image = (b1 - b0,) + tuple(p.image[1:])
+        return s
     q = p[b0:b1]
     hl = getattr(p, "_hl", None)
     if hl is not None:
@@ -117,17 +122,25 @@
         pre = real[4] if len(real) > 4 else None
         bank = end_points.get("tem_bank") if tem_cached is None else None
         T = h0 * w0 + 1
+        rgb_rows = end_points.get("tem_rgb_rows")
+
+        def tem_images(front=None):
+            if rgb_rows is not None and ops.patch_operand_ok(rgb_rows[0], front):
+                return ops.patch_operand(*rgb_rows, front=front)
+            tem = end_points["tem_rgb"] if rgb_rows is None else ops.gather_rows(*rgb_rows)
+            return tem if front is None else torch.cat([front, tem])
+
         if tem_cached is None and pre is not None and levels is not None:
             alloc, nxt = pre
             Bn = nxt.shape[0]
-            both, _ = fe.forward_tokens(torch.cat([nxt, end_points["tem_rgb"]]), level_out=(alloc, 0), full_depth=None if bank is None else Bn)
+            both, _ = fe.forward_tokens(tem_images(nxt), level_out=(alloc, 0), full_depth=None if bank is None else Bn)
             tem_tok = [t[Bn:] for t in both]
             if bank is not None:
                 nT = tem_tok[0].shape[0]
                 tem_tok[-1] = ops.bank_rows_to_tokens(*bank, T, out=alloc[-1][Bn * T:(Bn + nT) * T]).view(nT, T, -1)
             self._query_stash = (_tensor_key(nxt, fe), [a[:Bn * T].clone() for a in alloc], (h0, w0), nxt)
         elif tem_cached is None:
-            tem_tok, _ = fe.forward_tokens(end_points["tem_rgb"], level_out=None if levels is None else (levels, 0),
+            tem_tok, _ = fe.forward_tokens(tem_images(), level_out=None if levels is None else (levels, 0),
                                            full_depth=None if bank is None else 0)
             if bank is not None:
                 nT = tem_tok[0].shape[0]
@@ -148,7 +161,7 @@
         orr = self.offset_regressor
         if levels is not None and real_dpt is None and tem_cached is None:
             nT, nR = tem_tok[0].shape[0], levels[0].shape[0] // T - tem_tok[0].shape[0]
-            both = orr.dpt_head.forward_nhwc([as_img(lv.view(-1, T, lv.shape[1])) for lv in levels])
+            both = orr.dpt_head.forward_nhwc([as_img(lv.view(-1, T, lv.shape[1])) for lv in levels], finest_operand_only=True)
             tem_dpt, real_dpt = [_image_rows(p_, 0, nT) for p_ in both], [_image_rows(p_, nT, nT + nR) for p_ in both]
         else:
             if real_dpt is None:
@@ -187,9 +200,15 @@
         N = end_points["tem_pose"].shape[1]
         trow = rows if tidx is None else tidx[rows]
         flat = trow * N + idx
+        rgb_rows = None
+        if (ops.patch_operand_on() and not self.training and cache is None and levels is not None and end_points["tem_rgb"].dim() == 5
+                and end_points["tem_rgb"].is_contiguous() and flat.dtype == torch.int64 and ops.patch_operand_ok(end_points["tem_rgb"].flatten(0, 1))):
+            rgb_rows = (end_points["tem_rgb"].flatten(0, 1), flat)
         sel = {key: (ops.gather_rows(end_points[key].flatten(0, 1), flat) if end_points[key].is_contiguous()
                      else end_points[key][trow, idx])
-               for key in ("tem_pose", "tem_K", "tem_M", "tem_mask", "tem_rgb", "tem_pts3d")}
+               for key in ("tem_pose", "tem_K", "tem_M", "tem_mask", "tem_rgb", "tem_pts3d") if not (key == "tem_rgb" and rgb_rows is not None)}
+        if rgb_rows is not None:
+            sel["tem_rgb_rows"] = rgb_rows
         if self._last_from_bank(end_points):
             sel["tem_bank"] = (end_points["template_feature"].flatten(0, 1), flat)
         for key in ("real_pts2d", "real_K", "real_M", "real_mask", "real_pose"):
```

After: 581.0, median of 6. 2.2% higher.
